# REEVALUATE/knowledge_enhanced_multimodal_retrieval

Measured on AMD Instinct MI355X. Metric: gallery images+texts encoded/sec (ViT-L/14; synthetic texts per SURVEY 8(d): end-of-text uniform in positions 8..76, mean 43.8 of 77 positions computed -- value_every_text_77_positions is the rate when every text fills the context) and 43k x Q sim+top-10 ms, higher is better.
Workload: dtype bf16; 1 GPU; CLIP ViT-L/14 zero-shot: 43k-gallery encode (1 image + query + target text per item, 224x224 / 77 tokens) + T2I top-10, BASELINE configs[1]; architecture=ViT-L/14, residual_stream=fp24, batch_per_gpu=255, text_group=1501, gallery=43000, parallelism=dp1 (gallery sharded), rccl_ranks=1

## Files before the change

include/kemr_debug.h:

```cpp
#ifndef KEMR_DEBUG_H_
#define KEMR_DEBUG_H_

#include <stddef.h>
#include <stdint.h>

#ifdef __cplusplus
extern "C" {
#endif

int kemr_debug_set(const char* key, int value);
int kemr_debug_get(const char* key, int* value);

int kemr_debug_sim_lists(const void* workspace_dev, int nq, int ng, int64_t kdim, int k, int32_t* out6);

int kemr_debug_gemm_stamps(unsigned* host_out, int n_words);

int kemr_debug_op_attention_packed(const void* qkv_dev, void* out_dev, const int* row_start_dev, int batch, int max_t, int width,
                                   void* stream);
int kemr_debug_op_attention_pooled(const void* q_dev, const void* qkv_dev, void* out_dev, const int* pool_idx_dev,
                                   const int* row_start_dev, int items, int tokens, int width, int causal, int force_long, void* stream);
int kemr_debug_op_tail(const void* x_dev, int x_dtype, const void* delta_dev, const void* delta2_dev, const int32_t* ids_dev,
                       const int* row_start_dev, int batch, int tokens, int width, const float* gamma_dev, const float* beta_dev,
                       const float* proj_dev, int d, int normalize, float* out_dev, void* stream);

int kemr_debug_image_tokens(struct kemr_model* m, const float* pixels_dev, int batch, float* out_dev, void* workspace_dev,
                            size_t workspace_bytes, void* stream);
int kemr_debug_text_tokens(struct kemr_model* m, const int32_t* ids_dev, const int32_t* lens_dev, int rows, int batch, void* out_dev,
                           int* row_start_out_dev, void* workspace_dev, size_t workspace_bytes, void* stream);

#ifdef __cplusplus
}
#endif
#endif
```

knowledge_enhanced_multimodal_retrieval_amd/_lib.py:

```python
from __future__ import annotations

import ctypes as C
import os
import threading

PKG_DIR = os.path.dirname(os.path.abspath(__file__))
LIB_PATH = os.path.join(PKG_DIR, "libkemr.so")

KEMR_F32, KEMR_BF16, KEMR_I32, KEMR_FP8 = 0, 1, 2, 3
KEMR_F24 = 24
PREC_BF16 = 1
PREC_BF16_RES16 = 2
PREC_FP8 = 3
PREC_FP8_MLP = 4
PREC_FP8_RES16 = 5
DEFAULT_PRECISION = "bf16-x24"
PRECISIONS = {"bf16": PREC_BF16, "bf16-res16": PREC_BF16_RES16, "fp8": PREC_FP8, "fp8-mlp": PREC_FP8_MLP, "fp8-res16": PREC_FP8_RES16,
              "bf16-x24": PREC_BF16, "fp8-x24": PREC_FP8}
TOWER_VISION, TOWER_TEXT = 0, 1
SIDE_QUERY, SIDE_GALLERY = 0, 1
EPI_BIAS_BF16, EPI_BIAS_QGELU_BF16, EPI_BIAS_RESID_F32 = 0, 1, 2
EPI_BIAS_RESADD_BF16 = 4
MAX_DEEP_K = 1024


class KemrCfg(C.Structure):
    _fields_ = [(n, C.c_int32) for n in ("embed_dim", "image_size", "patch", "v_width", "v_layers",
                                          "t_width", "t_layers", "vocab", "ctx")]


_vp, _i, _i64, _f, _sz = C.c_void_p, C.c_int, C.c_int64, C.c_float, C.c_size_t

SIGNATURES = {
    "kemr_last_error": (C.c_char_p, []),
    "kemr_abi_version": (_i, []),
    "kemr_model_create": (_i, [C.POINTER(KemrCfg), C.POINTER(_vp)]),
    "kemr_model_load_tensor": (_i, [_vp, C.c_char_p, _vp, _i, C.POINTER(_i64), _i]),
    "kemr_model_finalize": (_i, [_vp, _i]),
    "kemr_model_destroy": (_i, [_vp]),
    "kemr_model_set_option": (_i, [_vp, C.c_char_p, _i]),
    "kemr_model_get_option": (_i, [_vp, C.c_char_p, C.POINTER(_i)]),
    "kemr_model_num_tensors": (_i, [_vp]),
    "kemr_model_tensor_name": (C.c_char_p, [_vp, _i]),
    "kemr_workspace_bytes": (_sz, [_vp, _i, _i]),
    "kemr_encode_image": (_i, [_vp, _vp, _i, _vp, _i, _vp, _sz, _vp]),
    "kemr_encode_text": (_i, [_vp, _vp, _i, _vp, _i, _vp, _sz, _vp]),
    "kemr_text_packed_workspace_bytes": (_sz, [_vp, _i, _i]),
    "kemr_encode_text_packed": (_i, [_vp, _vp, _vp, _i, _i, _vp, _i, _vp, _sz, _vp]),
    "kemr_panel_kdim": (_i64, [_i, _i, _i]),
    "kemr_panel_build": (_i, [C.POINTER(_vp), C.POINTER(_f), C.POINTER(_vp), _i, _i, _i, _i, _i, _vp, _vp]),
    "kemr_sim_workspace_bytes": (_sz, [_i, _i, _i64, _i]),
    "kemr_sim_topk": (_i, [_vp, _i, _vp, _i, _i64, _i64, _i, _vp, _vp, _vp, _vp, _vp, _vp, _vp, _vp, _vp, _sz, _vp]),
    "kemr_pair_scores": (_i, [_vp, _vp, _i64, _vp, _vp, _i, _vp, _vp]),
    "kemr_topk_merge": (_i, [_vp, _vp, _i, _i, _i, _vp, _vp, _vp]),
    "kemr_scores_dense": (_i, [_vp, _i, _vp, _i, _i64, _vp, _i64, _vp]),
    "kemr_rank_dense": (_i, [_vp, _i, _i, _i64, _vp, _vp, _i, _vp, _vp, _vp]),
    "kemr_select_topk": (_i, [_vp, _vp, _i, _i, _i64, _i64, _i, _vp, _vp, _vp]),
    "kemr_sim_topk_deep_workspace_bytes": (_sz, [_i, _i, _i64, _i]),
    "kemr_sim_topk_deep": (_i, [_vp, _i, _vp, _i, _i64, _i64, _i, _vp, _vp, _vp, _sz, _vp]),
    "kemr_sim_topk_deep_fused": (_i, [_vp, _i, _vp, _i, _i64, _i64, _i, _vp, _vp, _vp, _vp, _vp, _vp, _vp, _vp, _vp, _sz, _vp]),
    "kemr_linear_head": (_i, [_vp, _vp, _i64, _vp, _vp, _vp, _f, _i, _vp, _vp]),
    "kemr_gate_rows": (_i, [_vp, _i, _i, _vp, _vp, _f, _i, _vp, _vp]),
    "kemr_cross_attention_pairs": (_i, [_vp, _vp, _vp, _vp, _vp, _vp, _vp, _vp, _f, _i, _i, _i, _i, _i, _vp, _vp]),
    "kemr_cross_attention_rerank": (_i, [_vp, _vp, _vp, _vp, _vp, _vp, _vp, _vp, _vp, _f, _i, _i, _i, _i, _i, _i, _vp, _i, _i64, _vp, _vp]),
    "kemr_profile_begin": (_i, [_i]),
    "kemr_profile_end": (_i, [C.POINTER(C.c_double), C.POINTER(_i64), _i]),
    "kemr_op_gemm": (_i, [_vp, _vp, _vp, _vp, _i, _i, _i, _i, _vp]),
    "kemr_preprocess_workspace_bytes": (_sz, [_i, _i, _i]),
    "kemr_preprocess_u8": (_i, [_vp, _i, _i, _i, _vp, _vp, _sz, _vp]),
    "kemr_preprocess_batch_workspace_bytes": (_sz, [_vp, _vp, _i, _i]),
    "kemr_preprocess_u8_batch": (_i, [_vp, _vp, _vp, _vp, _i, _i, _vp, _vp, _sz, _vp]),
    "kemr_op_gemm_fp8": (_i, [_vp, _vp, _vp, _vp, _vp, _i, _i, _i, _i, _vp]),
    "kemr_op_e4m3_host": (_i, [_vp, _vp, C.c_longlong]),
    "kemr_op_layernorm": (_i, [_vp, _vp, _vp, _vp, _i, _i, _i, _vp]),
    "kemr_op_layernorm_resid": (_i, [_vp, _vp, _vp, _vp, _vp, _i, _i, _vp]),
    "kemr_op_layernorm_rows": (_i, [_vp, _i, _vp, _vp, _i, _vp, _vp, _vp, _i, _i, _i, _vp]),
    "kemr_op_attention": (_i, [_vp, _vp, _i, _i, _i, _i, _vp]),
}

DEBUG_SIGNATURES = {
    "kemr_debug_set": (_i, [C.c_char_p, _i]),
    "kemr_debug_get": (_i, [C.c_char_p, C.POINTER(_i)]),
    "kemr_debug_sim_lists": (_i, [_vp, _i, _i, _i64, _i, _vp]),
    "kemr_debug_gemm_stamps": (_i, [_vp, _i]),
    "kemr_debug_op_attention_packed": (_i, [_vp, _vp, _vp, _i, _i, _i, _vp]),
    "kemr_debug_op_attention_pooled": (_i, [_vp, _vp, _vp, _vp, _vp, _i, _i, _i, _i, _i, _vp]),
    "kemr_debug_op_tail": (_i, [_vp, _i, _vp, _vp, _vp, _vp, _i, _i, _i, _vp, _vp, _vp, _i, _i, _vp, _vp]),
    "kemr_debug_image_tokens": (_i, [_vp, _vp, _i, _vp, _vp, _sz, _vp]),
    "kemr_debug_text_tokens": (_i, [_vp, _vp, _vp, _i, _i, _vp, _vp, _vp, _sz, _vp]),
}
ABI_VERSION = 4

_lock = threading.Lock()
_lib = None


def lib() -> C.CDLL:
    global _lib
    if _lib is not None:
        return _lib
    with _lock:
        if _lib is not None:
            return _lib
        if not os.path.exists(LIB_PATH):
            raise RuntimeError(
                f"{LIB_PATH} is missing: build it with `python -m knowledge_enhanced_multimodal_retrieval_amd.build` "
                "(hipcc, gfx950). There is no CPU fallback for this path.")
        import torch
        handle = C.CDLL(LIB_PATH)
        for name, (res, args) in list(SIGNATURES.items()) + list(DEBUG_SIGNATURES.items()):
            try:
                fn = getattr(handle, name)
            except AttributeError as e:
                raise RuntimeError(f"{LIB_PATH} does not export {name}; rebuild the library") from e
            fn.restype = res
            fn.argtypes = args
        if handle.kemr_abi_version() != ABI_VERSION:
            raise RuntimeError(f"libkemr.so ABI version {handle.kemr_abi_version()} != {ABI_VERSION}; rebuild the library")
        _lib = handle
        return _lib


def check(status: int, what: str = "") -> None:
    if status != 0:
        msg = lib().kemr_last_error()
        raise RuntimeError(f"libkemr {what} failed ({status}): {msg.decode() if msg else '?'}")
```

knowledge_enhanced_multimodal_retrieval_amd/csrc/api.hip:

```cpp
#include "common.h"
#include "../../include/kemr_debug.h"

#include <cmath>
#include <cstdarg>
#include <cstdio>
#include <cstring>
#include <map>
#include <string>
#include <vector>

namespace kemr {

static thread_local char g_err[512] = "";
void set_error(const char* fmt, ...) {
    va_list ap;
    va_start(ap, fmt);
    vsnprintf(g_err, sizeof(g_err), fmt, ap);
    va_end(ap);
}

struct ProfState {
    bool on = false;
    std::vector<hipEvent_t> ev;
    std::vector<int> cls;
    int used = 0;
};
static ProfState g_prof;

ProfScope::ProfScope(int c, hipStream_t s) : slot(-1), stream(s) {
    if (!g_prof.on || g_prof.used >= (int)g_prof.cls.size()) return;
    slot = g_prof.used++;
    g_prof.cls[slot] = c;
    (void)hipEventRecord(g_prof.ev[2 * slot], stream);
}
ProfScope::~ProfScope() {
    if (slot >= 0) (void)hipEventRecord(g_prof.ev[2 * slot + 1], stream);
}

struct HostTensor {
    std::vector<int64_t> shape;
    std::vector<float> data;
    bool loaded = false;
};

struct LayerW {
    const float *ln1_g, *ln1_b, *ln2_g, *ln2_b, *bqkv, *bo, *b1, *b2;
    const bf16_t *wqkv, *wo, *w1, *w2;
    const uint8_t *wqkv8 = nullptr, *w18 = nullptr;
    const float *sqkv = nullptr, *s1 = nullptr;
};

struct TowerW {
    int width = 0, layers = 0, tokens = 0;
    std::vector<LayerW> layer;
};

}

using namespace kemr;

struct kemr_model {
    kemr_cfg cfg;
    std::vector<std::string> names;
    std::map<std::string, HostTensor> tensors;
    bool finalized = false;
    char* arena = nullptr;
    size_t arena_bytes = 0;
    int grid = 0, patches = 0, kpad = 0;
    int res_dtype = KEMR_F32;
    int fp8 = 0;
    int resadd = 1;
    int last_pooled = 1;
    int stream24 = 1;
    TowerW vis;
    const bf16_t* conv_w = nullptr;
    const float *cls = nullptr, *vpos = nullptr, *lnpre_g = nullptr, *lnpre_b = nullptr, *lnpost_g = nullptr,
                *lnpost_b = nullptr, *vproj = nullptr;
    TowerW txt;
    const float *tok = nullptr, *tpos = nullptr, *lnf_g = nullptr, *lnf_b = nullptr, *tproj = nullptr;
};

namespace {

void add_block_names(std::vector<std::string>& v, std::map<std::string, HostTensor>& t, const std::string& prefix,
                     int width, int layers) {
    auto add = [&](const std::string& n, std::vector<int64_t> shape) { v.push_back(n); t[n].shape = std::move(shape); };
    for (int i = 0; i < layers; ++i) {
        const std::string b = prefix + ".resblocks." + std::to_string(i);
        add(b + ".ln_1.weight", {width});
        add(b + ".ln_1.bias", {width});
        add(b + ".attn.in_proj_weight", {3 * width, width});
        add(b + ".attn.in_proj_bias", {3 * width});
        add(b + ".attn.out_proj.weight", {width, width});
        add(b + ".attn.out_proj.bias", {width});
        add(b + ".ln_2.weight", {width});
        add(b + ".ln_2.bias", {width});
        add(b + ".mlp.c_fc.weight", {4 * width, width});
        add(b + ".mlp.c_fc.bias", {4 * width});
        add(b + ".mlp.c_proj.weight", {width, 4 * width});
        add(b + ".mlp.c_proj.bias", {width});
    }
}

int check_cfg(const kemr_cfg& c) {
    if (c.embed_dim <= 0 || c.embed_dim > 1024) KEMR_FAIL(KEMR_ERR_INVALID, "cfg: embed_dim %d not in 1..1024", c.embed_dim);
    if (c.patch <= 0 || c.image_size <= 0 || c.image_size % c.patch) KEMR_FAIL(KEMR_ERR_INVALID, "cfg: image_size %% patch != 0");
    if (c.v_width % 256 || c.t_width % 256 || c.v_width <= 0 || c.t_width <= 0 || c.v_width > 1280 || c.t_width > 1280)
        KEMR_FAIL(KEMR_ERR_INVALID, "cfg: widths must be multiples of 256 in 256..1280 (got %d, %d)", c.v_width, c.t_width);
    if (c.v_layers <= 0 || c.t_layers <= 0 || c.vocab <= 0 || c.ctx <= 0) KEMR_FAIL(KEMR_ERR_INVALID, "cfg: non-positive field");
    const int g = c.image_size / c.patch;
    if (c.ctx > KEMR_MAX_TEXT_CTX) KEMR_FAIL(KEMR_ERR_INVALID, "cfg: sequence length > 288 not supported");
    if ((int64_t)g * g + 1 > KEMR_MAX_VISION_TOKENS)
        KEMR_FAIL(KEMR_ERR_INVALID, "cfg: vision sequence length %lld > %d not supported", (long long)g * g + 1, KEMR_MAX_VISION_TOKENS);
    const int kpad = (int)round_up(3 * c.patch * c.patch, 64);
    if (kpad > 4 * c.v_width) KEMR_FAIL(KEMR_ERR_INVALID, "cfg: patch too large for the workspace layout");
    return KEMR_OK;
}

struct ArenaPlan {
    size_t bytes = 0;
    size_t take(size_t n) { size_t o = bytes; bytes += (size_t)round_up((int64_t)n, 256); return o; }
};

}

extern "C" const char* kemr_last_error(void) { return g_err; }
extern "C" int kemr_abi_version(void) { return KEMR_ABI_VERSION; }

extern "C" int kemr_model_create(const kemr_cfg* cfg, kemr_model** out) {
    if (!cfg || !out) KEMR_FAIL(KEMR_ERR_INVALID, "model_create: null argument");
    KEMR_TRY(check_cfg(*cfg));
    kemr_model* m = new (std::nothrow) kemr_model();
    if (!m) KEMR_FAIL(KEMR_ERR_NOMEM, "model_create: out of memory");
    m->cfg = *cfg;
    { const char* v = getenv("KEMR_RESADD"); const int e = (v && *v) ? atoi(v) : 1; m->resadd = e < 0 ? 0 : e > 2 ? 2 : e; }
    { const char* v = getenv("KEMR_LAST_BLOCK_FULL"); m->last_pooled = (v && *v && atoi(v) != 0) ? 0 : 1; }
    { const char* v = getenv("KEMR_STREAM24"); m->stream24 = (v && *v) ? (atoi(v) != 0 ? 1 : 0) : 1; }
    m->grid = cfg->image_size / cfg->patch;
    m->patches = m->grid * m->grid;
    m->kpad = (int)round_up(3 * cfg->patch * cfg->patch, 64);
    auto add = [&](const std::string& n, std::vector<int64_t> shape) { m->names.push_back(n); m->tensors[n].shape = std::move(shape); };
    const int vw = cfg->v_width, tw = cfg->t_width, D = cfg->embed_dim;
    add("visual.conv1.weight", {vw, 3, cfg->patch, cfg->patch});
    add("visual.class_embedding", {vw});
    add("visual.positional_embedding", {m->patches + 1, vw});
    add("visual.ln_pre.weight", {vw});
    add("visual.ln_pre.bias", {vw});
    add_block_names(m->names, m->tensors, "visual.transformer", vw, cfg->v_layers);
    add("visual.ln_post.weight", {vw});
    add("visual.ln_post.bias", {vw});
    add("visual.proj", {vw, D});
    add("token_embedding.weight", {cfg->vocab, tw});
    add("positional_embedding", {cfg->ctx, tw});
    add_block_names(m->names, m->tensors, "transformer", tw, cfg->t_layers);
    add("ln_final.weight", {tw});
    add("ln_final.bias", {tw});
    add("text_projection", {tw, D});
    *out = m;
    return KEMR_OK;
}

extern "C" int kemr_model_num_tensors(const kemr_model* m) { return m ? (int)m->names.size() : 0; }
extern "C" const char* kemr_model_tensor_name(const kemr_model* m, int i) {
    if (!m || i < 0 || i >= (int)m->names.size()) return nullptr;
    return m->names[i].c_str();
}

extern "C" int kemr_model_load_tensor(kemr_model* m, const char* name, const void* host_ptr, int dtype,
                                      const int64_t* shape, int rank) {
    if (!m || !name || !host_ptr || (!shape && rank > 0)) KEMR_FAIL(KEMR_ERR_INVALID, "load_tensor: null argument");
    if (dtype != KEMR_F32) KEMR_FAIL(KEMR_ERR_INVALID, "load_tensor(%s): only fp32 host tensors are accepted", name);
    const std::string n(name);
    if (n == "logit_scale" || n == "input_resolution" || n == "context_length" || n == "vocab_size") return KEMR_OK;
    auto it = m->tensors.find(n);
    if (it == m->tensors.end()) KEMR_FAIL(KEMR_ERR_INVALID, "load_tensor: unexpected key '%s' (strict load)", name);
    HostTensor& t = it->second;
    bool same = (int)t.shape.size() == rank;
    int64_t numel = 1;
    for (int i = 0; same && i < rank; ++i) same = t.shape[i] == shape[i];
    if (!same) {
        std::string want, got;
        for (auto s : t.shape) want += std::to_string(s) + ",";
        for (int i = 0; i < rank; ++i) got += std::to_string(shape[i]) + ",";
        KEMR_FAIL(KEMR_ERR_INVALID, "load_tensor: size mismatch for %s: expected [%s] got [%s]", name, want.c_str(), got.c_str());
    }
    for (auto s : t.shape) numel *= s;
    t.data.assign((const float*)host_ptr, (const float*)host_ptr + numel);
    t.loaded = true;
    m->finalized = false;
    return KEMR_OK;
}

extern "C" int kemr_model_finalize(kemr_model* m, int precision) {
    if (!m) KEMR_FAIL(KEMR_ERR_INVALID, "finalize: null model");
    if (precision < KEMR_PREC_BF16 || precision > KEMR_PREC_FP8_RES16)
        KEMR_FAIL(KEMR_ERR_INVALID, "finalize: unsupported precision %d", precision);
    const int fp8 = (precision == KEMR_PREC_FP8 || precision == KEMR_PREC_FP8_RES16) ? 1 : precision == KEMR_PREC_FP8_MLP ? 3 : 0;
    if (fp8 && ((m->cfg.v_width % 128) || (m->cfg.t_width % 128) || m->cfg.v_width < 256 || m->cfg.t_width < 256))
        KEMR_FAIL(KEMR_ERR_INVALID, "finalize: fp8 needs tower widths that are multiples of 128 and >= 256");
    for (const auto& n : m->names)
        if (!m->tensors[n].loaded) KEMR_FAIL(KEMR_ERR_STATE, "finalize: missing key '%s' (strict load)", n.c_str());

    ArenaPlan plan;
    std::map<std::string, size_t> off;
    auto is_matrix = [](const std::string& n) {
        return n.find("in_proj_weight") != std::string::npos || n.find("out_proj.weight") != std::string::npos ||
               n.find("c_fc.weight") != std::string::npos || n.find("c_proj.weight") != std::string::npos ||
               n == "visual.conv1.weight";
    };
    auto is_fp8_matrix = [&](const std::string& n) {
        if (n.rfind("visual.", 0) != 0) return false;
        return ((fp8 & 1) && n.find("in_proj_weight") != std::string::npos) || ((fp8 & 2) && n.find("c_fc.weight") != std::string::npos);
    };
    for (const auto& n : m->names) {
        const HostTensor& t = m->tensors[n];
        size_t bytes;
        if (n == "visual.conv1.weight") bytes = (size_t)m->cfg.v_width * m->kpad * 2;
        else if (is_fp8_matrix(n)) { bytes = t.data.size(); off[n + "#scale"] = plan.take((size_t)t.shape[0] * 4); }
        else if (is_matrix(n)) bytes = t.data.size() * 2;
        else bytes = t.data.size() * 4;
        off[n] = plan.take(bytes);
    }
    auto ends_with = [](const std::string& a, const char* suf) { const size_t k = strlen(suf); return a.size() >= k && !a.compare(a.size() - k, k, suf); };
    auto ln_of = [&](const std::string& n) -> std::string {
        const size_t p = n.find(".attn.in_proj_weight");
        if (p != std::string::npos) return n.substr(0, p) + ".ln_1";
        const size_t q = n.find(".mlp.c_fc.weight");
        return q != std::string::npos ? n.substr(0, q) + ".ln_2" : std::string();
    };
    std::map<std::string, std::vector<float>> a_scale;
    if (fp8)
        for (const auto& n : m->names)
            if (is_fp8_matrix(n)) {
                const std::string ln = ln_of(n);
                const std::vector<float>&g = m->tensors[ln + ".weight"].data, &bb = m->tensors[ln + ".bias"].data;
                std::vector<float> sc(g.size(), 1.0f);
                for (size_t c = 0; c < g.size(); ++c) {
                    const float a = fmaxf(fabsf(g[c]), fabsf(bb[c]));
                    if (a > 0.f && std::isfinite(a)) sc[c] = exp2f(fminf(12.f, fmaxf(-12.f, ceilf(log2f(a)))));
                }
                a_scale[ln] = sc;
            }
    std::vector<char> host(plan.bytes, 0);
    for (const auto& n : m->names) {
        const HostTensor& t = m->tensors[n];
        char* dst = host.data() + off[n];
        if (n == "visual.conv1.weight") {
            const int kv = 3 * m->cfg.patch * m->cfg.patch;
            bf16_t* d = (bf16_t*)dst;
            for (int r = 0; r < m->cfg.v_width; ++r)
                for (int k = 0; k < kv; ++k) d[(size_t)r * m->kpad + k] = f32_to_bf16_host(t.data[(size_t)r * kv + k]);
        } else if (is_fp8_matrix(n)) {
            const int64_t rows = t.shape[0], cols = t.shape[1];
            const bool qkv = n.find("in_proj_weight") != std::string::npos;
            const std::vector<float>& as = a_scale.at(ln_of(n));
            uint8_t* d = (uint8_t*)dst;
            float* sc = (float*)(host.data() + off[n + "#scale"]);
            for (int64_t r = 0; r < rows; ++r) {
                const float pre = (qkv && r < cols) ? 0.125f : 1.0f;
                float amax = 0.f;
                for (int64_t c = 0; c < cols; ++c) amax = fmaxf(amax, fabsf(t.data[r * cols + c] * pre * as[c]));
                const float scale = amax > 0.f ? amax / 448.f : 1.0f;
                sc[r] = scale;
                for (int64_t c = 0; c < cols; ++c) d[r * cols + c] = f32_to_e4m3_host(t.data[r * cols + c] * pre * as[c] / scale);
            }
        } else if (n.find("in_proj_weight") != std::string::npos) {
            const int64_t w = t.shape[1];
            bf16_t* d = (bf16_t*)dst;
            for (int64_t i = 0; i < (int64_t)t.data.size(); ++i)
                d[i] = f32_to_bf16_host(i < w * w ? t.data[i] * 0.125f : t.data[i]);
        } else if (n.find("in_proj_bias") != std::string::npos) {
            const int64_t w = t.shape[0] / 3;
            float* d = (float*)dst;
            for (int64_t i = 0; i < (int64_t)t.data.size(); ++i) d[i] = i < w ? t.data[i] * 0.125f : t.data[i];
        } else if (is_matrix(n)) {
            bf16_t* d = (bf16_t*)dst;
            for (size_t i = 0; i < t.data.size(); ++i) d[i] = f32_to_bf16_host(t.data[i]);
        } else if (fp8 && (ends_with(n, ".ln_1.weight") || ends_with(n, ".ln_1.bias") || ends_with(n, ".ln_2.weight") || ends_with(n, ".ln_2.bias")) &&
                   a_scale.count(n.substr(0, n.rfind('.')))) {
            const std::vector<float>& as = a_scale.at(n.substr(0, n.rfind('.')));
            float* d = (float*)dst;
            for (size_t c = 0; c < t.data.size(); ++c) d[c] = t.data[c] / as[c];
        } else {
            memcpy(dst, t.data.data(), t.data.size() * 4);
        }
    }
    if (m->arena && m->arena_bytes != plan.bytes) { (void)hipFree(m->arena); m->arena = nullptr; }
    if (!m->arena) {
        KEMR_CHECK_HIP(hipMalloc((void**)&m->arena, plan.bytes));
        m->arena_bytes = plan.bytes;
    }
    KEMR_CHECK_HIP(hipDeviceSynchronize());
    KEMR_CHECK_HIP(hipMemcpy(m->arena, host.data(), plan.bytes, hipMemcpyHostToDevice));

    auto F = [&](const std::string& n) { return (const float*)(m->arena + off.at(n)); };
    auto H = [&](const std::string& n) { return (const bf16_t*)(m->arena + off.at(n)); };
    auto tower = [&](TowerW& tw, const std::string& prefix, int width, int layers, int tokens, int fp8) {
        tw.width = width; tw.layers = layers; tw.tokens = tokens;
        tw.layer.resize(layers);
        for (int i = 0; i < layers; ++i) {
            const std::string b = prefix + ".resblocks." + std::to_string(i);
            LayerW& L = tw.layer[i];
            L.ln1_g = F(b + ".ln_1.weight"); L.ln1_b = F(b + ".ln_1.bias");
            L.wqkv = H(b + ".attn.in_proj_weight"); L.bqkv = F(b + ".attn.in_proj_bias");
            if (fp8 & 1) { L.wqkv8 = (const uint8_t*)L.wqkv; L.wqkv = nullptr; L.sqkv = F(b + ".attn.in_proj_weight#scale"); }
            if (fp8 & 2) { L.w18 = (const uint8_t*)H(b + ".mlp.c_fc.weight"); L.s1 = F(b + ".mlp.c_fc.weight#scale"); }
            L.wo = H(b + ".attn.out_proj.weight"); L.bo = F(b + ".attn.out_proj.bias");
            L.ln2_g = F(b + ".ln_2.weight"); L.ln2_b = F(b + ".ln_2.bias");
            L.w1 = (fp8 & 2) ? nullptr : H(b + ".mlp.c_fc.weight"); L.b1 = F(b + ".mlp.c_fc.bias");
            L.w2 = H(b + ".mlp.c_proj.weight"); L.b2 = F(b + ".mlp.c_proj.bias");
        }
    };
    tower(m->vis, "visual.transformer", m->cfg.v_width, m->cfg.v_layers, m->patches + 1, fp8);
    tower(m->txt, "transformer", m->cfg.t_width, m->cfg.t_layers, m->cfg.ctx, 0);
    m->conv_w = H("visual.conv1.weight");
    m->cls = F("visual.class_embedding"); m->vpos = F("visual.positional_embedding");
    m->lnpre_g = F("visual.ln_pre.weight"); m->lnpre_b = F("visual.ln_pre.bias");
    m->lnpost_g = F("visual.ln_post.weight"); m->lnpost_b = F("visual.ln_post.bias");
    m->vproj = F("visual.proj");
    m->tok = F("token_embedding.weight"); m->tpos = F("positional_embedding");
    m->lnf_g = F("ln_final.weight"); m->lnf_b = F("ln_final.bias"); m->tproj = F("text_projection");

    for (auto& kv : m->tensors) { std::vector<float>().swap(kv.second.data); kv.second.loaded = false; }
    m->res_dtype = (precision == KEMR_PREC_BF16_RES16 || precision == KEMR_PREC_FP8_RES16) ? KEMR_BF16 : KEMR_F32;
    if (m->stream24 && m->res_dtype == KEMR_F32) m->res_dtype = KEMR_F24;
    m->fp8 = fp8;
    m->finalized = true;
    return KEMR_OK;
}

extern "C" int kemr_model_destroy(kemr_model* m) {
    if (!m) return KEMR_OK;
    if (m->arena) (void)hipFree(m->arena);
    delete m;
    return KEMR_OK;
}

namespace {

struct Workspace {
    void* x;
    int x_dtype;
    bf16_t* h;
    bf16_t* big;
    bf16_t* delta;
    bf16_t* delta2;
    float* x32;
    int* pool_idx;
    void* xc;
    bf16_t *hc, *qc, *ac, *d1c, *d2c;
    bf16_t* gc;
};

size_t compact_bytes(int width, int items) {
    const int64_t Mc = round_up((int64_t)items, 256);
    return (size_t)(round_up((int64_t)items * 4, 256) + Mc * width * 4 + 5 * Mc * width * 2 + Mc * width * 8);
}

size_t ws_bytes_rows(int width, int64_t rows, int x_dtype) {
    const int64_t Mp = round_up(rows, 256);
    const int xb = x_dtype == KEMR_BF16 ? 2 : (x_dtype == KEMR_F24 ? 3 : 4);
    return (size_t)(round_up(Mp * width * xb, 256) + 3 * round_up(Mp * width * 2, 256) + round_up(Mp * width * 8, 256));
}

size_t ws_bytes(int width, int tokens, int batch, int x_dtype) {
    const int64_t Mp = round_up((int64_t)batch * tokens, 256);
    const int xb = x_dtype == KEMR_BF16 ? 2 : (x_dtype == KEMR_F24 ? 3 : 4);
    return (size_t)(round_up(Mp * width * xb, 256) + 3 * round_up(Mp * width * 2, 256) + round_up(Mp * width * 8, 256));
}

int carve(Workspace& w, void* base, size_t bytes, int width, int64_t rows, int items, int x_dtype) {
    const size_t need = ws_bytes_rows(width, rows, x_dtype) + compact_bytes(width, items);
    if (!base || bytes < need) KEMR_FAIL(KEMR_ERR_WORKSPACE, "workspace too small: %zu < %zu bytes", bytes, need);
    if ((uintptr_t)base % 256) KEMR_FAIL(KEMR_ERR_WORKSPACE, "workspace must be 256-byte aligned");
    const int64_t Mp = round_up(rows, 256);
    char* p = (char*)base;
    w.x = p; w.x_dtype = x_dtype; p += round_up(Mp * width * (x_dtype == KEMR_BF16 ? 2 : (x_dtype == KEMR_F24 ? 3 : 4)), 256);
    w.x32 = x_dtype == KEMR_F32 ? (float*)w.x : (float*)p;
    w.h = (bf16_t*)p; p += round_up(Mp * width * 2, 256);
    w.delta = (bf16_t*)p; p += round_up(Mp * width * 2, 256);
    w.delta2 = (bf16_t*)p; p += round_up(Mp * width * 2, 256);
    w.big = (bf16_t*)p; p += round_up(Mp * width * 8, 256);
    const int64_t Mc = round_up((int64_t)items, 256);
    w.pool_idx = (int*)p; p += round_up((int64_t)items * 4, 256);
    w.xc = p; p += Mc * width * 4;
    w.hc = (bf16_t*)p; p += Mc * width * 2;
    w.qc = (bf16_t*)p; p += Mc * width * 2;
    w.ac = (bf16_t*)p; p += Mc * width * 2;
    w.d1c = (bf16_t*)p; p += Mc * width * 2;
    w.d2c = (bf16_t*)p; p += Mc * width * 2;
    w.gc = (bf16_t*)p;
    return KEMR_OK;
}

int run_blocks(const TowerW& t, const Workspace& w, int batch, int causal, int fp8, int want_resadd, hipStream_t s, bool* pending,
               const int* row_start = nullptr, int rows = 0, int last_pooled = 0, const int32_t* ids = nullptr, bool* compact = nullptr) {
    const int W = t.width, M = row_start ? rows : batch * t.tokens;
    const bool fq = fp8 & 1, f1 = fp8 & 2;
    bool resadd = want_resadd >= (w.x_dtype == KEMR_BF16 ? 1 : 2) && M > 512 && W % 256 == 0 && w.x_dtype != KEMR_F24;
    const int cs = w.x_dtype == KEMR_BF16 ? 2 : 4;
    const int epi_res = w.x_dtype == KEMR_BF16 ? EPI_BIAS_RESADD_BF16 : EPI_BIAS_RESID_F32;
    if (resadd) {
        GemmParams a{}, b{};
        a.M = b.M = M; a.N = b.N = W; a.K = W; b.K = 4 * W; a.lda = W; b.lda = 4 * W; a.ldw = W; b.ldw = 4 * W; a.ldc = b.ldc = W;
        a.c_rows_padded = b.c_rows_padded = 1;
        resadd = gemm256u_fits(a, 2, cs) && gemm256u_fits(b, 2, cs);
    }
    *pending = !resadd && t.layers > 0;
    const bool pooled = last_pooled && compact && !resadd && !f1 && t.layers > 0 && t.tokens <= KEMR_MAX_VISION_TOKENS;
    if (compact) *compact = pooled;
    if (pooled) KEMR_TRY(launch_pool_index(causal ? ids : nullptr, row_start, batch, t.tokens, w.pool_idx, s));
    for (int l = 0; l < t.layers; ++l) {
        const LayerW& L = t.layer[l];
        if (pooled && l == t.layers - 1) {
            KEMR_TRY(launch_layernorm(w.x, w.x_dtype, l ? w.delta : nullptr, l ? w.delta2 : nullptr, 1, L.ln1_g, L.ln1_b, w.h, M, W, fq ? KEMR_FP8 : KEMR_BF16, s));
            GemmParams g{};
            g.c_rows_padded = 1;
            g.M = M; g.A = w.h; g.lda = W; g.ldw = W; g.bias = L.bqkv + W; g.C = w.big + W; g.ldc = 3 * W; g.N = 2 * W; g.K = W;
            if (fq) { g.W = (const bf16_t*)(L.wqkv8 + (size_t)W * W); g.wscale = L.sqkv + W; KEMR_TRY(launch_gemm256u_fp8(g, EPI_BIAS_BF16, s)); }
            else { g.W = L.wqkv + (size_t)W * W; KEMR_TRY(launch_gemm(g, EPI_BIAS_BF16, s)); }
            KEMR_TRY(launch_gather_pooled(w.x, w.x_dtype, w.h, fq ? KEMR_FP8 : KEMR_BF16, w.pool_idx, batch, W, w.xc, w.hc, s));
            g.M = batch; g.A = w.hc; g.bias = L.bqkv; g.C = w.qc; g.ldc = W; g.N = W;
            if (fq) { g.W = (const bf16_t*)L.wqkv8; g.wscale = L.sqkv; KEMR_TRY(launch_gemm256u_fp8(g, EPI_BIAS_BF16, s)); g.wscale = nullptr; }
            else { g.W = L.wqkv; KEMR_TRY(launch_gemm(g, EPI_BIAS_BF16, s)); }
            KEMR_TRY(launch_attention_pooled(w.qc, w.big, w.ac, w.pool_idx, row_start, batch, t.tokens, W, causal, s));
            g.A = w.ac; g.W = L.wo; g.bias = L.bo; g.C = w.d1c;
            KEMR_TRY(launch_gemm(g, EPI_BIAS_BF16, s));
            KEMR_TRY(launch_layernorm(w.xc, w.x_dtype, w.d1c, nullptr, 0, L.ln2_g, L.ln2_b, w.hc, batch, W, KEMR_BF16, s));
            g.A = w.hc; g.W = L.w1; g.bias = L.b1; g.C = w.gc; g.ldc = 4 * W; g.N = 4 * W;
            KEMR_TRY(launch_gemm(g, EPI_BIAS_QGELU_BF16, s));
            g.A = w.gc; g.lda = 4 * W; g.W = L.w2; g.ldw = 4 * W; g.bias = L.b2; g.C = w.d2c; g.ldc = W; g.N = W; g.K = 4 * W;
            KEMR_TRY(launch_gemm(g, EPI_BIAS_BF16, s));
            break;
        }
        if (resadd) KEMR_TRY(launch_layernorm(w.x, w.x_dtype, nullptr, nullptr, 0, L.ln1_g, L.ln1_b, w.h, M, W, fq ? KEMR_FP8 : KEMR_BF16, s));
        else KEMR_TRY(launch_layernorm(w.x, w.x_dtype, l ? w.delta : nullptr, l ? w.delta2 : nullptr, 1, L.ln1_g, L.ln1_b, w.h, M, W, fq ? KEMR_FP8 : KEMR_BF16, s));
        GemmParams g{};
        g.M = M;
        g.c_rows_padded = 1;
        g.A = w.h; g.lda = W; g.W = L.wqkv; g.ldw = W; g.bias = L.bqkv; g.C = w.big; g.ldc = 3 * W; g.N = 3 * W; g.K = W;
        if (fq) {
            g.W = (const bf16_t*)L.wqkv8; g.wscale = L.sqkv;
            KEMR_TRY(launch_gemm256u_fp8(g, EPI_BIAS_BF16, s));
            g.wscale = nullptr;
        } else {
            KEMR_TRY(launch_gemm(g, EPI_BIAS_BF16, s));
        }
        if (row_start) KEMR_TRY(launch_attention_packed(w.big, w.h, row_start, batch, t.tokens, W, s));
        else KEMR_TRY(launch_attention(w.big, w.h, batch, t.tokens, W, causal, s));
        g.A = w.h; g.lda = W; g.W = L.wo; g.ldw = W; g.bias = L.bo; g.C = resadd ? w.x : (void*)w.delta; g.ldc = W; g.N = W; g.K = W;
        KEMR_TRY(launch_gemm(g, resadd ? epi_res : EPI_BIAS_BF16, s));
        KEMR_TRY(launch_layernorm(w.x, w.x_dtype, resadd ? nullptr : w.delta, nullptr, 0, L.ln2_g, L.ln2_b, w.h, M, W, f1 ? KEMR_FP8 : KEMR_BF16, s));
        g.A = w.h; g.lda = W; g.W = L.w1; g.ldw = W; g.bias = L.b1; g.C = w.big; g.ldc = 4 * W; g.N = 4 * W; g.K = W;
        if (f1) {
            g.W = (const bf16_t*)L.w18; g.wscale = L.s1;
            KEMR_TRY(launch_gemm256u_fp8(g, EPI_BIAS_QGELU_BF16, s));
            g.wscale = nullptr;
        } else {
            KEMR_TRY(launch_gemm(g, EPI_BIAS_QGELU_BF16, s));
        }
        g.A = w.big; g.lda = 4 * W; g.W = L.w2; g.ldw = 4 * W; g.bias = L.b2; g.C = resadd ? w.x : (void*)w.delta2; g.ldc = W; g.N = W; g.K = 4 * W;
        KEMR_TRY(launch_gemm(g, resadd ? epi_res : EPI_BIAS_BF16, s));
    }
    return KEMR_OK;
}

int image_front(kemr_model* m, const float* pixels_dev, int batch, const void* out_dev, void* workspace_dev, size_t workspace_bytes,
                hipStream_t s, const char* what, Workspace& w) {
    if (!m || !pixels_dev || !out_dev) KEMR_FAIL(KEMR_ERR_INVALID, "%s: null argument", what);
    if (!m->finalized) KEMR_FAIL(KEMR_ERR_STATE, "%s: model not finalized", what);
    if (batch <= 0) return batch == 0 ? KEMR_OK : (set_error("%s: negative batch", what), KEMR_ERR_INVALID);
    if ((int64_t)batch * (m->patches + 1) > (1 << 24)) KEMR_FAIL(KEMR_ERR_INVALID, "%s: batch %d too large", what, batch);
    const int W = m->cfg.v_width, T = m->patches + 1;
    KEMR_TRY(carve(w, workspace_dev, workspace_bytes, W, (int64_t)batch * T, batch, m->res_dtype));
    KEMR_TRY(launch_im2col(pixels_dev, w.big, batch, m->cfg.image_size, m->cfg.patch, m->kpad, s));
    GemmParams g{};
    g.A = w.big; g.lda = m->kpad; g.W = m->conv_w; g.ldw = m->kpad; g.bias = nullptr; g.C = w.x32; g.ldc = W;
    g.pos = m->vpos; g.patches = m->patches; g.M = batch * m->patches; g.N = W; g.K = m->kpad;
    KEMR_TRY(launch_gemm(g, EPI_PATCH_F32, s));
    return launch_cls_rows(w.x32, m->cls, m->vpos, batch, T, W, s);
}

int text_front(kemr_model* m, const int32_t* ids_dev, const int32_t* lens_dev, int rows, int batch, bool packed, const void* out_dev,
               void* workspace_dev, size_t workspace_bytes, hipStream_t s, const char* what, Workspace& w, int** row_start) {
    if (!m || !ids_dev || !out_dev || (packed && !lens_dev)) KEMR_FAIL(KEMR_ERR_INVALID, "%s: null argument", what);
    if (!m->finalized) KEMR_FAIL(KEMR_ERR_STATE, "%s: model not finalized", what);
    if (batch <= 0) return batch == 0 ? KEMR_OK : (set_error("%s: negative batch", what), KEMR_ERR_INVALID);
    if ((int64_t)batch * m->cfg.ctx > (1 << 24)) KEMR_FAIL(KEMR_ERR_INVALID, "%s: batch %d too large", what, batch);
    const int W = m->cfg.t_width, T = m->cfg.ctx;
    *row_start = nullptr;
    if (!packed) {
        KEMR_TRY(carve(w, workspace_dev, workspace_bytes, W, (int64_t)batch * T, batch, m->res_dtype));
        return launch_text_embed(ids_dev, m->tok, m->tpos, w.x, w.x_dtype, batch, T, W, m->cfg.vocab, s);
    }
    if (m->cfg.ctx > 128) KEMR_FAIL(KEMR_ERR_INVALID, "%s: context length %d > 128", what, m->cfg.ctx);
    if (rows < batch || (int64_t)rows > (int64_t)batch * T) KEMR_FAIL(KEMR_ERR_INVALID, "%s: %d rows for %d texts of 1 .. %d positions", what, rows, batch, T);
    const size_t base_bytes = ws_bytes_rows(W, rows, m->res_dtype) + compact_bytes(W, batch), need = base_bytes + (size_t)round_up(((int64_t)batch + 1) * 4, 256);
    if (workspace_bytes < need) KEMR_FAIL(KEMR_ERR_WORKSPACE, "workspace too small: %zu < %zu bytes", workspace_bytes, need);
    KEMR_TRY(carve(w, workspace_dev, workspace_bytes, W, rows, batch, m->res_dtype));
    *row_start = (int*)((char*)workspace_dev + base_bytes);
    KEMR_TRY(launch_row_starts(lens_dev, batch, T, rows, *row_start, s));
    return launch_text_embed(ids_dev, m->tok, m->tpos, w.x, w.x_dtype, batch, T, W, m->cfg.vocab, s, *row_start, rows);
}

}

extern "C" size_t kemr_workspace_bytes(const kemr_model* m, int tower, int batch) {
    if (!m || batch <= 0) return 0;
    if (tower == KEMR_TOWER_VISION) return ws_bytes(m->cfg.v_width, m->patches + 1, batch, m->res_dtype) + compact_bytes(m->cfg.v_width, batch);
    if (tower == KEMR_TOWER_TEXT) return ws_bytes(m->cfg.t_width, m->cfg.ctx, batch, m->res_dtype) + compact_bytes(m->cfg.t_width, batch);
    return 0;
}

extern "C" size_t kemr_text_packed_workspace_bytes(const kemr_model* m, int rows, int batch) {
    if (!m || batch <= 0 || rows < batch) return 0;
    return ws_bytes_rows(m->cfg.t_width, rows, m->res_dtype) + compact_bytes(m->cfg.t_width, batch) +
           (size_t)round_up(((int64_t)batch + 1) * 4, 256);
}

extern "C" int kemr_encode_image(kemr_model* m, const float* pixels_dev, int batch, float* out_dev, int normalize,
                                 void* workspace_dev, size_t workspace_bytes, void* stream) {
    hipStream_t s = (hipStream_t)stream;
    Workspace w;
    KEMR_TRY(image_front(m, pixels_dev, batch, out_dev, workspace_dev, workspace_bytes, s, "encode_image", w));
    if (batch == 0) return KEMR_OK;
    const int W = m->cfg.v_width, T = m->patches + 1;
    KEMR_TRY(launch_layernorm(w.x32, KEMR_F32, nullptr, nullptr, 0, m->lnpre_g, m->lnpre_b, w.x, batch * T, W, w.x_dtype, s));
    bool vb = false, vc = false;
    KEMR_TRY(run_blocks(m->vis, w, batch, 0, m->fp8, m->resadd, s, &vb, nullptr, 0, m->last_pooled, nullptr, &vc));
    if (vc) KEMR_TRY(launch_tail(w.xc, w.x_dtype, w.d1c, w.d2c, nullptr, batch, 1, W, m->lnpost_g, m->lnpost_b, m->vproj, m->cfg.embed_dim, normalize, out_dev, s));
    else KEMR_TRY(launch_tail(w.x, w.x_dtype, vb ? w.delta : nullptr, vb ? w.delta2 : nullptr, nullptr, batch, T, W, m->lnpost_g, m->lnpost_b, m->vproj, m->cfg.embed_dim, normalize, out_dev, s));
    return KEMR_OK;
}

extern "C" int kemr_encode_text(kemr_model* m, const int32_t* ids_dev, int batch, float* out_dev, int normalize,
                                void* workspace_dev, size_t workspace_bytes, void* stream) {
    hipStream_t s = (hipStream_t)stream;
    Workspace w;
    int* no_rows = nullptr;
    KEMR_TRY(text_front(m, ids_dev, nullptr, 0, batch, false, out_dev, workspace_dev, workspace_bytes, s, "encode_text", w, &no_rows));
    if (batch == 0) return KEMR_OK;
    const int W = m->cfg.t_width, T = m->cfg.ctx;
    bool tb = false, tc = false;
    KEMR_TRY(run_blocks(m->txt, w, batch, 1, 0, m->resadd, s, &tb, nullptr, 0, m->last_pooled, ids_dev, &tc));
    if (tc) KEMR_TRY(launch_tail(w.xc, w.x_dtype, w.d1c, w.d2c, nullptr, batch, 1, W, m->lnf_g, m->lnf_b, m->tproj, m->cfg.embed_dim, normalize, out_dev, s));
    else KEMR_TRY(launch_tail(w.x, w.x_dtype, tb ? w.delta : nullptr, tb ? w.delta2 : nullptr, ids_dev, batch, T, W, m->lnf_g, m->lnf_b, m->tproj, m->cfg.embed_dim, normalize, out_dev, s));
    return KEMR_OK;
}

extern "C" int kemr_encode_text_packed(kemr_model* m, const int32_t* ids_dev, const int32_t* lens_dev, int rows, int batch, float* out_dev,
                                       int normalize, void* workspace_dev, size_t workspace_bytes, void* stream) {
    hipStream_t s = (hipStream_t)stream;
    Workspace w;
    int* row_start = nullptr;
    KEMR_TRY(text_front(m, ids_dev, lens_dev, rows, batch, true, out_dev, workspace_dev, workspace_bytes, s, "encode_text_packed", w, &row_start));
    if (batch == 0) return KEMR_OK;
    const int W = m->cfg.t_width, T = m->cfg.ctx;
    bool tb = false, tc = false;
    KEMR_TRY(run_blocks(m->txt, w, batch, 1, 0, m->resadd, s, &tb, row_start, rows, m->last_pooled, ids_dev, &tc));
    if (tc) KEMR_TRY(launch_tail(w.xc, w.x_dtype, w.d1c, w.d2c, nullptr, batch, 1, W, m->lnf_g, m->lnf_b, m->tproj, m->cfg.embed_dim, normalize, out_dev, s));
    else KEMR_TRY(launch_tail(w.x, w.x_dtype, tb ? w.delta : nullptr, tb ? w.delta2 : nullptr, ids_dev, batch, T, W, m->lnf_g, m->lnf_b, m->tproj, m->cfg.embed_dim, normalize, out_dev, s, row_start));
    return KEMR_OK;
}

extern "C" int kemr_model_set_option(kemr_model* m, const char* key, int value) {
    if (!m || !key) KEMR_FAIL(KEMR_ERR_INVALID, "model_set_option: null argument");
    if (!strcmp(key, "residual_fusion")) {
        if (value < 0 || value > 2) KEMR_FAIL(KEMR_ERR_INVALID, "model_set_option(residual_fusion): 0, 1 or 2, got %d", value);
        m->resadd = value;
        return KEMR_OK;
    }
    if (!strcmp(key, "residual_stream_24bit")) {
        if (value < 0 || value > 1) KEMR_FAIL(KEMR_ERR_INVALID, "model_set_option(residual_stream_24bit): 0 or 1, got %d", value);
        if (m->finalized) KEMR_FAIL(KEMR_ERR_STATE, "model_set_option(residual_stream_24bit): set it before kemr_model_finalize");
        m->stream24 = value;
        return KEMR_OK;
    }
    if (!strcmp(key, "last_block_pooled_row")) {
        if (value < 0 || value > 1) KEMR_FAIL(KEMR_ERR_INVALID, "model_set_option(last_block_pooled_row): 0 or 1, got %d", value);
        m->last_pooled = value;
        return KEMR_OK;
    }
    KEMR_FAIL(KEMR_ERR_INVALID, "model_set_option: unknown key '%s'", key);
}

extern "C" int kemr_model_get_option(const kemr_model* m, const char* key, int* value) {
    if (!m || !key || !value) KEMR_FAIL(KEMR_ERR_INVALID, "model_get_option: null argument");
    if (!strcmp(key, "residual_fusion")) { *value = m->resadd; return KEMR_OK; }
    if (!strcmp(key, "last_block_pooled_row")) { *value = m->last_pooled; return KEMR_OK; }
    if (!strcmp(key, "residual_stream_24bit")) { *value = m->finalized ? (m->res_dtype == KEMR_F24) : m->stream24; return KEMR_OK; }
    if (!strcmp(key, "precision_residual_bf16")) { *value = m->res_dtype == KEMR_BF16; return KEMR_OK; }
    KEMR_FAIL(KEMR_ERR_INVALID, "model_get_option: unknown key '%s'", key);
}

namespace {
#ifdef KEMR_AB_VARIANTS
int g_ab_variants = 1;
#else
int g_ab_variants = 0;
#endif
struct DebugKnob { const char* key; int* var; int lo, hi; unsigned product; };
int* sim_lists_knob();
const DebugKnob* debug_knobs(int* n) {
    static const DebugKnob knobs[] = {
        {"gemm_variant", &g_gemm_variant, 0, 9, 1u << 0 | 1u << 1 | 1u << 2 | 1u << 7 | 1u << 8},
        {"gemm_flags", &g_gemm_dbg, 0, 255, 1u << 0},
        {"gemm_order", &g_gemm_order, 0, 8, ~0u},
        {"gemm_grid", &g_gemm_grid, 0, 1024, ~0u},
        {"gemm_conc", &g_gemm_conc, 0, 2, ~0u},
        {"gemm_kl", &g_gemm_kl, 0, 1, 1u << 0},
        {"attn_v", &g_attn_v, 0, 5, 1u << 0},
        {"attn_xcd", &g_attn_xcd, 0, 1, ~0u},
        {"attn_waves", &g_attn_waves, 0, 8, 1u << 0},
        {"ln_nt", &g_ln_nt, 0, 3, 1u << 3},
        {"sim_lists", sim_lists_knob(), 0, 3, ~0u},
        {"ab_variants", &g_ab_variants, -1, -2, 0},
    };
    *n = (int)(sizeof(knobs) / sizeof(knobs[0]));
    return knobs;
}
int* sim_lists_knob() { return &g_sim_lists; }
}

extern "C" int kemr_debug_set(const char* key, int value) {
    if (!key) KEMR_FAIL(KEMR_ERR_INVALID, "debug_set: null key");
    int n = 0;
    const DebugKnob* k = debug_knobs(&n);
    for (int i = 0; i < n; ++i)
        if (!strcmp(k[i].key, key)) {
            if (k[i].lo > k[i].hi) KEMR_FAIL(KEMR_ERR_INVALID, "debug_set(%s): read-only", key);
            if (value < k[i].lo || value > k[i].hi) KEMR_FAIL(KEMR_ERR_INVALID, "debug_set(%s): %d not in %d..%d", key, value, k[i].lo, k[i].hi);
            if (!g_ab_variants && !(value < 32 && ((k[i].product >> value) & 1u)) && k[i].product != ~0u)
                KEMR_FAIL(KEMR_ERR_INVALID, "debug_set(%s): %d selects an A/B experiment kernel that is not in this library (build.py --ab-variants)", key, value);
            *k[i].var = value;
            return KEMR_OK;
        }
    KEMR_FAIL(KEMR_ERR_INVALID, "debug_set: unknown key '%s'", key);
}

extern "C" int kemr_debug_get(const char* key, int* value) {
    if (!key || !value) KEMR_FAIL(KEMR_ERR_INVALID, "debug_get: null argument");
    int n = 0;
    const DebugKnob* k = debug_knobs(&n);
    for (int i = 0; i < n; ++i)
        if (!strcmp(k[i].key, key)) { *value = *k[i].var; return KEMR_OK; }
    KEMR_FAIL(KEMR_ERR_INVALID, "debug_get: unknown key '%s'", key);
}

extern "C" int kemr_debug_gemm_stamps(unsigned* host_out, int n_words) {
    if (!host_out) KEMR_FAIL(KEMR_ERR_INVALID, "debug_gemm_stamps: null output");
    return gemm_read_stamps(host_out, n_words);
}

extern "C" int kemr_debug_op_attention_packed(const void* qkv_dev, void* out_dev, const int* row_start_dev, int batch, int max_t, int width,
                                              void* stream) {
    if (!qkv_dev || !out_dev) KEMR_FAIL(KEMR_ERR_INVALID, "debug_op_attention_packed: null argument");
    return launch_attention_packed((const bf16_t*)qkv_dev, (bf16_t*)out_dev, row_start_dev, batch, max_t, width, (hipStream_t)stream);
}

extern "C" int kemr_debug_op_attention_pooled(const void* q_dev, const void* qkv_dev, void* out_dev, const int* pool_idx_dev,
                                              const int* row_start_dev, int items, int tokens, int width, int causal, int force_long,
                                              void* stream) {
    if (!q_dev || !qkv_dev || !out_dev) KEMR_FAIL(KEMR_ERR_INVALID, "debug_op_attention_pooled: null argument");
    return launch_attention_pooled((const bf16_t*)q_dev, (const bf16_t*)qkv_dev, (bf16_t*)out_dev, pool_idx_dev, row_start_dev, items,
                                   tokens, width, causal, (hipStream_t)stream, force_long);
}

extern "C" int kemr_debug_op_tail(const void* x_dev, int x_dtype, const void* delta_dev, const void* delta2_dev, const int32_t* ids_dev,
                                  const int* row_start_dev, int batch, int tokens, int width, const float* gamma_dev, const float* beta_dev,
                                  const float* proj_dev, int d, int normalize, float* out_dev, void* stream) {
    if (!x_dev || !gamma_dev || !beta_dev || !proj_dev || !out_dev) KEMR_FAIL(KEMR_ERR_INVALID, "debug_op_tail: null argument");
    if (x_dtype != KEMR_F32 && x_dtype != KEMR_BF16 && x_dtype != KEMR_F24) KEMR_FAIL(KEMR_ERR_INVALID, "debug_op_tail: bad row dtype %d", x_dtype);
    return launch_tail(x_dev, x_dtype, (const bf16_t*)delta_dev, (const bf16_t*)delta2_dev, ids_dev, batch, tokens, width, gamma_dev, beta_dev,
                       proj_dev, d, normalize, out_dev, (hipStream_t)stream, row_start_dev);
}

extern "C" int kemr_debug_image_tokens(kemr_model* m, const float* pixels_dev, int batch, float* out_dev, void* workspace_dev,
                                       size_t workspace_bytes, void* stream) {
    hipStream_t s = (hipStream_t)stream;
    Workspace w;
    KEMR_TRY(image_front(m, pixels_dev, batch, out_dev, workspace_dev, workspace_bytes, s, "debug_image_tokens", w));
    if (batch == 0) return KEMR_OK;
    const size_t bytes = (size_t)batch * (m->patches + 1) * m->cfg.v_width * 4;
    KEMR_CHECK_HIP(hipMemcpyAsync(out_dev, w.x32, bytes, hipMemcpyDeviceToDevice, s));
    return KEMR_OK;
}

extern "C" int kemr_debug_text_tokens(kemr_model* m, const int32_t* ids_dev, const int32_t* lens_dev, int rows, int batch, void* out_dev,
                                      int* row_start_out_dev, void* workspace_dev, size_t workspace_bytes, void* stream) {
    const bool packed = lens_dev != nullptr;
    if (packed && !row_start_out_dev) KEMR_FAIL(KEMR_ERR_INVALID, "debug_text_tokens: null row_start output");
    hipStream_t s = (hipStream_t)stream;
    Workspace w;
    int* row_start = nullptr;
    KEMR_TRY(text_front(m, ids_dev, lens_dev, rows, batch, packed, out_dev, workspace_dev, workspace_bytes, s, "debug_text_tokens", w, &row_start));
    if (batch == 0) return KEMR_OK;
    const int xb = w.x_dtype == KEMR_BF16 ? 2 : (w.x_dtype == KEMR_F24 ? 3 : 4);
    const int64_t n = packed ? rows : (int64_t)batch * m->cfg.ctx;
    KEMR_CHECK_HIP(hipMemcpyAsync(out_dev, w.x, (size_t)n * m->cfg.t_width * xb, hipMemcpyDeviceToDevice, s));
    if (packed) KEMR_CHECK_HIP(hipMemcpyAsync(row_start_out_dev, row_start, ((size_t)batch + 1) * 4, hipMemcpyDeviceToDevice, s));
    return KEMR_OK;
}

extern "C" int kemr_profile_begin(int max_launches) {
    if (max_launches <= 0 || max_launches > (1 << 20)) KEMR_FAIL(KEMR_ERR_INVALID, "profile_begin: bad max_launches");
    if (g_prof.on) KEMR_FAIL(KEMR_ERR_STATE, "profile_begin: already profiling");
    while ((int)g_prof.ev.size() < 2 * max_launches) {
        hipEvent_t e;
        KEMR_CHECK_HIP(hipEventCreate(&e));
        g_prof.ev.push_back(e);
    }
    g_prof.cls.assign(max_launches, 0);
    g_prof.used = 0;
    g_prof.on = true;
    return KEMR_OK;
}

extern "C" int kemr_profile_end(double* ms_per_class, int64_t* launches_per_class, int nclass) {
    if (!g_prof.on) KEMR_FAIL(KEMR_ERR_STATE, "profile_end: not profiling");
    g_prof.on = false;
    if (!ms_per_class || !launches_per_class || nclass < PROF_NCLASS) KEMR_FAIL(KEMR_ERR_INVALID, "profile_end: need %d classes", PROF_NCLASS);
    for (int i = 0; i < nclass; ++i) { ms_per_class[i] = 0; launches_per_class[i] = 0; }
    KEMR_CHECK_HIP(hipDeviceSynchronize());
    for (int i = 0; i < g_prof.used; ++i) {
        float ms = 0.f;
        KEMR_CHECK_HIP(hipEventElapsedTime(&ms, g_prof.ev[2 * i], g_prof.ev[2 * i + 1]));
        ms_per_class[g_prof.cls[i]] += ms;
        launches_per_class[g_prof.cls[i]] += 1;
    }
    return KEMR_OK;
}

extern "C" int kemr_op_gemm(const void* a_dev, const void* w_dev, const float* bias_dev, void* c_dev, int m, int n, int k,
                            int epilogue, void* stream) {
    if (!a_dev || !w_dev || !c_dev) KEMR_FAIL(KEMR_ERR_INVALID, "op_gemm: null argument");
    if (epilogue < 0 || (epilogue > KEMR_EPI_BIAS_RESID_F32 && epilogue != KEMR_EPI_BIAS_RESADD_BF16)) KEMR_FAIL(KEMR_ERR_INVALID, "op_gemm: bad epilogue %d", epilogue);
    GemmParams g{};
    g.A = (const bf16_t*)a_dev; g.lda = k; g.W = (const bf16_t*)w_dev; g.ldw = k; g.bias = bias_dev; g.C = c_dev; g.ldc = n;
    g.M = m; g.N = n; g.K = k;
    g.c_rows_padded = 1;
    return launch_gemm(g, epilogue, (hipStream_t)stream);
}

extern "C" int kemr_op_gemm_fp8(const void* a_dev, const void* w_dev, const float* wscale_dev, const float* bias_dev, void* c_dev,
                                int m, int n, int k, int epilogue, void* stream) {
    if (!a_dev || !w_dev || !wscale_dev || !c_dev) KEMR_FAIL(KEMR_ERR_INVALID, "op_gemm_fp8: null argument");
    GemmParams g{};
    g.A = (const bf16_t*)a_dev; g.lda = k; g.W = (const bf16_t*)w_dev; g.ldw = k; g.bias = bias_dev; g.wscale = wscale_dev;
    g.C = c_dev; g.ldc = n; g.M = m; g.N = n; g.K = k;
    g.c_rows_padded = 1;
    return launch_gemm256u_fp8(g, epilogue, (hipStream_t)stream);
}

extern "C" int kemr_op_e4m3_host(const float* in, unsigned char* out, long long n) {
    if (!in || !out || n < 0) KEMR_FAIL(KEMR_ERR_INVALID, "op_e4m3_host: bad argument");
    for (long long i = 0; i < n; ++i) out[i] = f32_to_e4m3_host(in[i]);
    return KEMR_OK;
}

extern "C" int kemr_op_layernorm(const float* x_dev, const float* gamma_dev, const float* beta_dev, void* y_dev, int rows,
                                 int width, int out_dtype, void* stream) {
    if (!x_dev || !gamma_dev || !beta_dev || !y_dev) KEMR_FAIL(KEMR_ERR_INVALID, "op_layernorm: null argument");
    return launch_layernorm((void*)x_dev, KEMR_F32, nullptr, nullptr, 0, gamma_dev, beta_dev, y_dev, rows, width, out_dtype, (hipStream_t)stream);
}

extern "C" int kemr_op_layernorm_resid(float* x_dev, const void* delta_dev, const float* gamma_dev, const float* beta_dev,
                                       void* y_dev, int rows, int width, void* stream) {
    if (!x_dev || !delta_dev || !gamma_dev || !beta_dev || !y_dev) KEMR_FAIL(KEMR_ERR_INVALID, "op_layernorm_resid: null argument");
    return launch_layernorm(x_dev, KEMR_F32, (const bf16_t*)delta_dev, nullptr, 1, gamma_dev, beta_dev, y_dev, rows, width, KEMR_BF16, (hipStream_t)stream);
}

extern "C" int kemr_op_layernorm_rows(void* x_dev, int x_dtype, const void* delta_dev, const void* delta2_dev, int writeback,
                                      const float* gamma_dev, const float* beta_dev, void* y_dev, int rows, int width,
                                      int out_dtype, void* stream) {
    if (!x_dev || !gamma_dev || !beta_dev || !y_dev) KEMR_FAIL(KEMR_ERR_INVALID, "op_layernorm_rows: null argument");
    return launch_layernorm(x_dev, x_dtype, (const bf16_t*)delta_dev, (const bf16_t*)delta2_dev, writeback, gamma_dev, beta_dev,
                            y_dev, rows, width, out_dtype, (hipStream_t)stream);
}

extern "C" int kemr_op_attention(const void* qkv_dev, void* out_dev, int batch, int t, int width, int causal, void* stream) {
    if (!qkv_dev || !out_dev) KEMR_FAIL(KEMR_ERR_INVALID, "op_attention: null argument");
    return launch_attention((const bf16_t*)qkv_dev, (bf16_t*)out_dev, batch, t, width, causal, (hipStream_t)stream);
}
```

knowledge_enhanced_multimodal_retrieval_amd/csrc/attention.hip:

```cpp
#include "common.h"

namespace kemr {

__device__ __forceinline__ bf16x4 lds_read_tr16(const char* p) {
    typedef __attribute__((ext_vector_type(4))) short s4;
    return __builtin_amdgcn_ds_read_tr16_b64_v4i16((__attribute__((address_space(3))) s4*)p);
}

__device__ __forceinline__ bool attn_item(int xbatch, int& h, int& b) {
    h = blockIdx.x; b = blockIdx.y;
    if (xbatch == 0) return true;
    const int id = blockIdx.y * gridDim.x + blockIdx.x, j = id >> 3;
    b = (j / (int)gridDim.x) * 8 + (id & 7);
    h = j % (int)gridDim.x;
    return b < xbatch;
}

#ifndef KEMR_ATTN_PRIO
#define KEMR_ATTN_PRIO 0
#endif
__device__ __forceinline__ void attn_prio(int mfma_phase) {
    if constexpr (KEMR_ATTN_PRIO == 1) { if (mfma_phase) __builtin_amdgcn_s_setprio(1); else __builtin_amdgcn_s_setprio(0); }
    if constexpr (KEMR_ATTN_PRIO == 2) { if (mfma_phase) __builtin_amdgcn_s_setprio(0); else __builtin_amdgcn_s_setprio(1); }
}

template <bool NT>
__device__ __forceinline__ bf16x8 load_q8(const bf16_t* p) {
    if constexpr (NT) return __builtin_nontemporal_load((const bf16x8*)p);
    else return *(const bf16x8*)p;
}

template <int NT32, bool CAUSAL, int TC, int NW = 4, bool STAMP = false, int NTLOAD = 1, bool SKIPTAIL = false>
__global__ __launch_bounds__(NW * 64, 2) void attention_kernel(const bf16_t* __restrict__ qkv, bf16_t* __restrict__ out,
                                                           int T_rt, int width, int xbatch, const int* __restrict__ row_start) {
    constexpr int TP = NT32 * 32;
    constexpr int NT16 = NT32 * 2;
    constexpr int NTH = NW * 64;
    constexpr int NCH = (TP * 8 + NTH - 1) / NTH;
    constexpr float LOG2E = 1.4426950408889634f;
    extern __shared__ __attribute__((aligned(16))) char smem[];
    char* sK = smem;
    char* sV = smem + TP * 128;

    int h, b;
    if (!attn_item(xbatch, h, b)) return;
    int T_ = TC > 0 ? TC : T_rt;
    size_t row0 = (size_t)b * T_;
    if (TC == 0 && row_start) {
        const int r0 = row_start[b];
        T_ = row_start[b + 1] - r0;
        row0 = r0;
    }
    const int T = T_;
    const int tid = threadIdx.x, lane = tid & 63;
    const int wid = __builtin_amdgcn_readfirstlane(tid >> 6);
    const int ld = 3 * width;
    const bf16_t* base = qkv + row0 * ld + h * 64;
    const int lrow = lane & 15, lq = lane >> 4;
    const int nqt = SKIPTAIL ? T >> 4 : (T + 15) >> 4;

    unsigned long long st_t[8] = {0, 0, 0, 0, 0, 0, 0, 0}, st_prev = 0;
    auto stamp = [&](int k) {
        if constexpr (STAMP) {
            __builtin_amdgcn_sched_barrier(0);
            unsigned long long now;
            asm volatile("s_memtime %0\n\ts_waitcnt lgkmcnt(0)" : "=s"(now) :: "memory");
            __builtin_amdgcn_sched_barrier(0);
            st_t[k] += now - st_prev;
            st_prev = now;
        }
    };
    if constexpr (STAMP) { asm volatile("s_memtime %0\n\ts_waitcnt lgkmcnt(0)" : "=s"(st_prev) :: "memory"); __builtin_amdgcn_sched_barrier(0); }
    bf16x8 qn[2];
    {
        const int q0 = wid * 16 + lrow;
        const int qc = q0 < T ? q0 : T - 1;
#pragma unroll
        for (int kk = 0; kk < 2; ++kk) qn[kk] = load_q8<(NTLOAD >= 2)>(base + (size_t)qc * ld + kk * 32 + lq * 8);
    }
    {
        uint4 kv[NCH], vv[NCH];
#pragma unroll
        for (int i = 0; i < NCH; ++i) {
            const int idx = tid + i * NTH;
            const int row = idx >> 3, c = idx & 7;
            const int rc = row < T ? row : T - 1;
            if constexpr (NTLOAD >= 1) {
                typedef unsigned u32x4_ __attribute__((ext_vector_type(4)));
                const u32x4_ a_ = __builtin_nontemporal_load((const u32x4_*)(base + (size_t)rc * ld + width + c * 8));
                const u32x4_ b_ = __builtin_nontemporal_load((const u32x4_*)(base + (size_t)rc * ld + 2 * width + c * 8));
                kv[i] = make_uint4(a_.x, a_.y, a_.z, a_.w);
                vv[i] = make_uint4(b_.x, b_.y, b_.z, b_.w);
            } else {
                kv[i] = *(const uint4*)(base + (size_t)rc * ld + width + c * 8);
                vv[i] = *(const uint4*)(base + (size_t)rc * ld + 2 * width + c * 8);
            }
        }
#pragma unroll
        for (int i = 0; i < NCH; ++i) {
            const int idx = tid + i * NTH;
            const int row = idx >> 3, c = idx & 7;
            if (idx < TP * 8) {
                const unsigned keep = row < T ? 0xffffffffu : 0u;
                uint4 a = kv[i], b2 = vv[i];
                a.x &= keep; a.y &= keep; a.z &= keep; a.w &= keep;
                b2.x &= keep; b2.y &= keep; b2.z &= keep; b2.w &= keep;
                *(uint4*)(sK + row * 128 + ((c ^ ((row >> 1) & 7)) << 4)) = a;
                *(uint4*)(sV + row * 128 + ((c ^ (((row >> 1) & 3) << 1)) << 4)) = b2;
            }
        }
    }
    __syncthreads();
    stamp(0);

    for (int qt = wid; qt < nqt; qt += NW) {
        const int q = qt * 16 + lrow;
        bf16x8 qf[2] = {qn[0], qn[1]};
        if (qt + NW < nqt) {
            const int q2 = q + NW * 16;
            const int qc = q2 < T ? q2 : T - 1;
#pragma unroll
            for (int kk = 0; kk < 2; ++kk) qn[kk] = load_q8<(NTLOAD >= 2)>(base + (size_t)qc * ld + kk * 32 + lq * 8);
        }

        constexpr int G = (NT16 % 3 == 0) ? 3 : 2;
        constexpr int NG = NT16 / G;
        f32x4 s[NT16];
        bf16x8 kfr[2][G][2];
        auto load_group = [&](int g, bf16x8 (&dst)[G][2]) {
#pragma unroll
            for (int j = 0; j < G; ++j)
#pragma unroll
                for (int kk = 0; kk < 2; ++kk)
                    dst[j][kk] = *(const bf16x8*)(sK + ((g * G + j) * 16 + lrow) * 128 + (((kk * 4 + lq) ^ (lrow >> 1)) << 4));
        };
        load_group(0, kfr[0]);
        attn_prio(1);
#pragma unroll
        for (int g = 0; g < NG; ++g) {
            if (g + 1 < NG && (g + 1) * G * 16 < T) load_group(g + 1, kfr[(g + 1) & 1]);
            __builtin_amdgcn_sched_barrier(0);
#pragma unroll
            for (int j = 0; j < G; ++j) {
                const int t = g * G + j;
                s[t] = f32x4{0.f, 0.f, 0.f, 0.f};
                if (t * 16 < T && (!CAUSAL || t <= qt)) {
                    s[t] = __builtin_amdgcn_mfma_f32_16x16x32_bf16(kfr[g & 1][j][0], qf[0], s[t], 0, 0, 0);
                    s[t] = __builtin_amdgcn_mfma_f32_16x16x32_bf16(kfr[g & 1][j][1], qf[1], s[t], 0, 0, 0);
                }
            }
            __builtin_amdgcn_sched_barrier(0);
        }
        attn_prio(0);
        stamp(1);
        float mx = -INFINITY;
#pragma unroll
        for (int t = 0; t < NT16; ++t) {
            const bool partial = (t + 1) * 16 > T || CAUSAL;
#pragma unroll
            for (int r = 0; r < 4; ++r) {
                if (partial) {
                    const int key = t * 16 + lq * 4 + r;
                    const bool ok = key < T && (!CAUSAL || key <= q);
                    s[t][r] = ok ? s[t][r] : -INFINITY;
                }
                mx = fmaxf(mx, s[t][r]);
            }
        }
        mx = fmaxf(mx, __shfl_xor(mx, 16));
        mx = fmaxf(mx, __shfl_xor(mx, 32));
        const float mxl = mx * LOG2E;
        stamp(2);
        f32x2_t sum2 = {0.f, 0.f};
        const f32x2_t l2 = {LOG2E, LOG2E}, nm = {-mxl, -mxl};
        auto exp_tile = [&](int t) {
            f32x2_t a = f32x2_t{s[t][0], s[t][1]} * l2 + nm, c = f32x2_t{s[t][2], s[t][3]} * l2 + nm;
            a.x = __builtin_amdgcn_exp2f(a.x); a.y = __builtin_amdgcn_exp2f(a.y);
            c.x = __builtin_amdgcn_exp2f(c.x); c.y = __builtin_amdgcn_exp2f(c.y);
            s[t][0] = a.x; s[t][1] = a.y; s[t][2] = c.x; s[t][3] = c.y;
            sum2 += a;
            sum2 += c;
        };
#pragma unroll
        for (int t = 0; t < NT16; ++t) exp_tile(t);

        stamp(3);
        f32x4 o[4];
#pragma unroll
        for (int dt = 0; dt < 4; ++dt) o[dt] = f32x4{0.f, 0.f, 0.f, 0.f};
        bf16x8 vfr[2][4];
        auto load_v = [&](int u, bf16x8 (&dst)[4]) {
            const int ra = u * 32 + lq * 4 + (lrow >> 2);
            const int rb = ra + 16;
#pragma unroll
            for (int dt = 0; dt < 4; ++dt) {
                const int c = dt * 2 + ((lrow & 3) >> 1);
                const bf16x4 va = lds_read_tr16(sV + ra * 128 + ((c ^ (((ra >> 1) & 3) << 1)) << 4) + (lrow & 1) * 8);
                const bf16x4 vb = lds_read_tr16(sV + rb * 128 + ((c ^ (((rb >> 1) & 3) << 1)) << 4) + (lrow & 1) * 8);
                dst[dt][0] = va[0]; dst[dt][1] = va[1]; dst[dt][2] = va[2]; dst[dt][3] = va[3];
                dst[dt][4] = vb[0]; dst[dt][5] = vb[1]; dst[dt][6] = vb[2]; dst[dt][7] = vb[3];
            }
        };
        load_v(0, vfr[0]);
        attn_prio(1);
        auto live = [&](int u) { return u < NT32 && u * 32 < T && !(CAUSAL && u * 32 > qt * 16 + 15); };
#pragma unroll
        for (int u = 0; u < NT32; ++u) {
            if (!live(u)) continue;
            if (u + 1 < NT32 && (u + 1) * 32 < T) load_v(u + 1, vfr[(u + 1) & 1]);
            __builtin_amdgcn_sched_barrier(0);
            union { bf16x8 v; uint32_t w[4]; } pf;
            pf.w[0] = pack_bf16x2(s[2 * u][0], s[2 * u][1]);
            pf.w[1] = pack_bf16x2(s[2 * u][2], s[2 * u][3]);
            pf.w[2] = pack_bf16x2(s[2 * u + 1][0], s[2 * u + 1][1]);
            pf.w[3] = pack_bf16x2(s[2 * u + 1][2], s[2 * u + 1][3]);
#pragma unroll
            for (int dt = 0; dt < 4; ++dt)
                o[dt] = __builtin_amdgcn_mfma_f32_16x16x32_bf16(vfr[u & 1][dt], pf.v, o[dt], 0, 0, 0);
            __builtin_amdgcn_sched_barrier(0);
        }
        attn_prio(0);
        stamp(4);
        float sum = sum2.x + sum2.y;
        sum += __shfl_xor(sum, 16);
        sum += __shfl_xor(sum, 32);
        if (q < T) {
            const float inv = 1.0f / sum;
            bf16_t* dst = out + (row0 + q) * width + h * 64 + lq * 4;
#pragma unroll
            for (int dt = 0; dt < 4; ++dt) {
                uint2 pk;
                pk.x = pack_bf16x2(o[dt][0] * inv, o[dt][1] * inv);
                pk.y = pack_bf16x2(o[dt][2] * inv, o[dt][3] * inv);
                *(uint2*)(dst + dt * 16) = pk;
            }
        }
        stamp(5);
    }
    if constexpr (STAMP) {
        unsigned long long* dst = (unsigned long long*)(out + (size_t)xbatch * T * width) + (((size_t)b * (width >> 6) + h) * NW + wid) * 8;
        if (lane == 0) {
#pragma unroll
            for (int k = 0; k < 6; ++k) dst[k] += st_t[k];
            dst[6] += 1;
        }
    }
}

int g_attn_v = 0;

int g_attn_xcd = 1;
int g_attn_waves = 0;

#ifdef KEMR_AB_VARIANTS
int launch_attention_ab(int v, int waves, const bf16_t* qkv, bf16_t* out, int batch, int width, int xbatch, hipStream_t stream);
#endif

template <int NT32>
static int launch_nt(const bf16_t* qkv, bf16_t* out, int batch, int t, int width, int causal, hipStream_t stream, const int* row_start = nullptr) {
    constexpr int smem = NT32 * 32 * 128 * 2;
    const dim3 grid(width / 64, batch);
    ProfScope prof(PROF_ATTENTION, stream);
    void (*kern)(const bf16_t*, bf16_t*, int, int, int, const int*);
    const int xbatch = g_attn_xcd ? batch : 0;
    const dim3 xgrid(width / 64, xbatch ? (batch + 7) / 8 * 8 : batch);
    int threads = 256;
    if (causal) {
        if (NT32 == 3 && t == 77 && !row_start) { kern = attention_kernel<NT32, true, NT32 == 3 ? 77 : 0, NT32 == 3 ? 5 : 4>; threads = 320; }
        else kern = attention_kernel<NT32, true, 0>;
    } else if (NT32 == 9 && t == 257) {
#ifdef KEMR_AB_VARIANTS
        if (g_attn_v != 0) return launch_attention_ab(g_attn_v, g_attn_waves, qkv, out, batch, width, xbatch, stream);
        if (g_attn_waves == 6) { kern = attention_kernel<NT32, false, NT32 == 9 ? 257 : 0, NT32 == 9 ? 6 : 4>; threads = 384; }
        else if (g_attn_waves == 7) kern = attention_kernel<NT32, false, NT32 == 9 ? 257 : 0, 4, false, NT32 == 9 ? 0 : 1>;
        else if (g_attn_waves == 8) kern = attention_kernel<NT32, false, NT32 == 9 ? 257 : 0, 4, false, 1, NT32 == 9>;
        else if (g_attn_waves == 5) kern = attention_kernel<NT32, false, NT32 == 9 ? 257 : 0, 4, false, NT32 == 9 ? 2 : 1>;
        else if (g_attn_waves == 2 && xbatch) kern = attention_kernel<NT32, false, NT32 == 9 ? 257 : 0, 4, NT32 == 9>;
        else
#else
        if (g_attn_v != 0 || g_attn_waves != 0)
            KEMR_FAIL(KEMR_ERR_INVALID, "attention: attn_v = %d / attn_waves = %d select A/B kernels this library was built without (build.py --ab-variants)", g_attn_v, g_attn_waves);
#endif
        kern = attention_kernel<NT32, false, NT32 == 9 ? 257 : 0>;
    } else {
        kern = attention_kernel<NT32, false, 0>;
    }
    KEMR_CHECK_HIP(hipFuncSetAttribute((const void*)kern, hipFuncAttributeMaxDynamicSharedMemorySize, smem));
    hipLaunchKernelGGL(kern, xgrid, dim3(threads), smem, stream, qkv, out, t, width, xbatch, row_start);
    KEMR_CHECK_LAUNCH("attention_kernel");
    return KEMR_OK;
}

int launch_attention(const bf16_t* qkv, bf16_t* out, int batch, int t, int width, int causal, hipStream_t stream) {
    if (batch <= 0) return KEMR_OK;
    if (width % 64 != 0 || t <= 0) KEMR_FAIL(KEMR_ERR_INVALID, "attention: bad shape t=%d width=%d", t, width);
    if (batch > 65528) KEMR_FAIL(KEMR_ERR_INVALID, "attention: batch %d > 65528 (grid.y, rounded up to a multiple of 8)", batch);
    const int nt32 = (t + 31) / 32;
    switch (nt32) {
        case 1: return launch_nt<1>(qkv, out, batch, t, width, causal, stream);
        case 2: return launch_nt<2>(qkv, out, batch, t, width, causal, stream);
        case 3: return launch_nt<3>(qkv, out, batch, t, width, causal, stream);
        case 4: return launch_nt<4>(qkv, out, batch, t, width, causal, stream);
        case 5: return launch_nt<5>(qkv, out, batch, t, width, causal, stream);
        case 6: return launch_nt<6>(qkv, out, batch, t, width, causal, stream);
        case 7: return launch_nt<7>(qkv, out, batch, t, width, causal, stream);
        case 8: return launch_nt<8>(qkv, out, batch, t, width, causal, stream);
        case 9: return launch_nt<9>(qkv, out, batch, t, width, causal, stream);
    }
    if (!causal && t <= KEMR_MAX_VISION_TOKENS) return launch_attention_long(qkv, out, batch, t, width, stream);
    if (!causal) KEMR_FAIL(KEMR_ERR_INVALID, "attention: sequence length %d > %d not supported", t, KEMR_MAX_VISION_TOKENS);
    KEMR_FAIL(KEMR_ERR_INVALID, "attention: sequence length %d > 288 not supported (causal)", t);
}

__device__ __forceinline__ void wave_lds_fence() {
    __builtin_amdgcn_fence(__ATOMIC_RELEASE, "wavefront");
    __builtin_amdgcn_wave_barrier();
    __builtin_amdgcn_fence(__ATOMIC_ACQUIRE, "wavefront");
}

template <int MAXK>
__global__ __launch_bounds__(256) void attention_pooled_kernel(const bf16_t* __restrict__ q, const bf16_t* __restrict__ qkv,
                                                               bf16_t* __restrict__ out, const int* __restrict__ pool_idx,
                                                               const int* __restrict__ row_start, int items, int tokens, int width,
                                                               int causal) {
    constexpr float LOG2E = 1.4426950408889634f;
    __shared__ float sp[4][MAXK];
    const int heads = width >> 6, lane = threadIdx.x & 63, wv = threadIdx.x >> 6;
    const int item = blockIdx.x * 4 + wv;
    if (item >= items * heads) return;
    const int b = item / heads, h = item - b * heads;
    const int r0 = row_start ? row_start[b] : b * tokens;
    int nk = causal ? pool_idx[b] - r0 + 1 : tokens;
    nk = nk < 1 ? 1 : (nk > MAXK ? MAXK : nk);
    const size_t ld = 3 * (size_t)width;
    const int ck = lane & 7, kq = lane >> 3;
    float qf[8];
    {
        const uint4 v = ((const uint4*)(q + (size_t)b * width + h * 64))[ck];
        const uint32_t w4[4] = {v.x, v.y, v.z, v.w};
#pragma unroll
        for (int k = 0; k < 4; ++k) {
            qf[2 * k] = bf16_to_f32((bf16_t)(w4[k] & 0xffff));
            qf[2 * k + 1] = bf16_to_f32((bf16_t)(w4[k] >> 16));
        }
    }
    const bf16_t* kbase = qkv + (size_t)r0 * ld + width + h * 64 + ck * 8;
    const int npass = (nk + 7) >> 3;
    for (int pss = 0; pss < npass; ++pss) {
        const int j = pss * 8 + kq;
        const int jc = j < nk ? j : nk - 1;
        const uint4 v = *(const uint4*)(kbase + (size_t)jc * ld);
        const uint32_t w4[4] = {v.x, v.y, v.z, v.w};
        float s = 0.f;
#pragma unroll
        for (int k = 0; k < 4; ++k) {
            s = fmaf(qf[2 * k], bf16_to_f32((bf16_t)(w4[k] & 0xffff)), s);
            s = fmaf(qf[2 * k + 1], bf16_to_f32((bf16_t)(w4[k] >> 16)), s);
        }
        s += __shfl_xor(s, 1);
        s += __shfl_xor(s, 2);
        s += __shfl_xor(s, 4);
        if (ck == 0 && j < nk) sp[wv][j] = s;
    }
    wave_lds_fence();
    float sc[MAXK / 64];
    float mx = -INFINITY;
#pragma unroll
    for (int pss = 0; pss < MAXK / 64; ++pss) {
        const int j = pss * 64 + lane;
        sc[pss] = j < nk ? sp[wv][j] : -INFINITY;
        mx = fmaxf(mx, sc[pss]);
    }
#pragma unroll
    for (int o = 32; o > 0; o >>= 1) mx = fmaxf(mx, __shfl_xor(mx, o));
    float sum = 0.f;
#pragma unroll
    for (int pss = 0; pss < MAXK / 64; ++pss) {
        const int j = pss * 64 + lane;
        const float p = __builtin_amdgcn_exp2f((sc[pss] - mx) * LOG2E);
        sum += p;
        if (j < MAXK) sp[wv][j] = bf16_to_f32(f32_to_bf16(p));
    }
#pragma unroll
    for (int o = 32; o > 0; o >>= 1) sum += __shfl_xor(sum, o);
    wave_lds_fence();
    const int dp = lane & 31, par = lane >> 5;
    const bf16_t* vp = qkv + (size_t)r0 * ld + 2 * width + h * 64 + dp * 2;
    float a0 = 0.f, a1 = 0.f;
#pragma unroll 4
    for (int j = par; j < nk; j += 2) {
        const uint32_t v = *(const uint32_t*)(vp + (size_t)j * ld);
        const float p = sp[wv][j];
        a0 = fmaf(p, bf16_to_f32((bf16_t)(v & 0xffff)), a0);
        a1 = fmaf(p, bf16_to_f32((bf16_t)(v >> 16)), a1);
    }
    a0 += __shfl_xor(a0, 32);
    a1 += __shfl_xor(a1, 32);
    if (par == 0) {
        const float inv = 1.0f / sum;
        *(uint32_t*)(out + (size_t)b * width + h * 64 + dp * 2) = pack_bf16x2(a0 * inv, a1 * inv);
    }
}

int launch_attention_pooled(const bf16_t* q, const bf16_t* qkv, bf16_t* out, const int* pool_idx, const int* row_start, int items,
                            int tokens, int width, int causal, hipStream_t stream, int force_long) {
    if (items <= 0) return KEMR_OK;
    if (width % 64 != 0 || tokens <= 0 || tokens > KEMR_MAX_VISION_TOKENS)
        KEMR_FAIL(KEMR_ERR_INVALID, "attention (pooled row): bad shape t=%d width=%d", tokens, width);
    if (causal && !pool_idx) KEMR_FAIL(KEMR_ERR_INVALID, "attention (pooled row): the causal form needs the pooled positions");
    ProfScope prof(PROF_ATTENTION, stream);
    const long waves = (long)items * (width / 64);
    constexpr int MAXK_LONG = (KEMR_MAX_VISION_TOKENS + 63) / 64 * 64;
    void (*kern)(const bf16_t*, const bf16_t*, bf16_t*, const int*, const int*, int, int, int, int) =
        tokens <= 320 && !force_long ? attention_pooled_kernel<320> : attention_pooled_kernel<MAXK_LONG>;
    hipLaunchKernelGGL(kern, dim3((unsigned)((waves + 3) / 4)), dim3(256), 0, stream, q, qkv, out, pool_idx, row_start, items, tokens,
                       width, causal);
    KEMR_CHECK_LAUNCH("attention_pooled_kernel");
    return KEMR_OK;
}

int launch_attention_packed(const bf16_t* qkv, bf16_t* out, const int* row_start, int batch, int max_t, int width, hipStream_t stream) {
    if (batch <= 0) return KEMR_OK;
    if (!row_start) KEMR_FAIL(KEMR_ERR_INVALID, "attention: packed rows need row_start");
    if (width % 64 != 0 || max_t <= 0) KEMR_FAIL(KEMR_ERR_INVALID, "attention: bad shape t=%d width=%d", max_t, width);
    if (batch > 65528) KEMR_FAIL(KEMR_ERR_INVALID, "attention: batch %d > 65528 (grid.y, rounded up to a multiple of 8)", batch);
    switch ((max_t + 31) / 32) {
        case 1: return launch_nt<1>(qkv, out, batch, max_t, width, 1, stream, row_start);
        case 2: return launch_nt<2>(qkv, out, batch, max_t, width, 1, stream, row_start);
        case 3: return launch_nt<3>(qkv, out, batch, max_t, width, 1, stream, row_start);
        case 4: return launch_nt<4>(qkv, out, batch, max_t, width, 1, stream, row_start);
    }
    KEMR_FAIL(KEMR_ERR_INVALID, "attention: packed rows support lengths up to 128, got %d", max_t);
}

}
```

knowledge_enhanced_multimodal_retrieval_amd/csrc/common.h:

```cpp
#pragma once
#include <hip/hip_runtime.h>
#include <stdint.h>
#include <stddef.h>
#include "../../include/kemr.h"

namespace kemr {

typedef uint16_t bf16_t;
typedef __attribute__((ext_vector_type(8))) short bf16x8;
typedef __attribute__((ext_vector_type(4))) short bf16x4;
typedef __attribute__((ext_vector_type(4))) float f32x4;

void set_error(const char* fmt, ...);
#define KEMR_FAIL(code, ...) do { ::kemr::set_error(__VA_ARGS__); return (code); } while (0)
#define KEMR_CHECK_HIP(expr) do { hipError_t e_ = (expr); if (e_ != hipSuccess) { \
    ::kemr::set_error("%s failed: %s (%s:%d)", #expr, hipGetErrorString(e_), __FILE__, __LINE__); \
    return KEMR_ERR_HIP; } } while (0)
#define KEMR_CHECK_LAUNCH(what) do { hipError_t e_ = hipGetLastError(); if (e_ != hipSuccess) { \
    ::kemr::set_error("launch of %s failed: %s (%s:%d)", what, hipGetErrorString(e_), __FILE__, __LINE__); \
    return KEMR_ERR_HIP; } } while (0)
#define KEMR_TRY(expr) do { int r_ = (expr); if (r_ != KEMR_OK) return r_; } while (0)

static inline uint16_t f32_to_bf16_host(float f) {
    uint32_t u; __builtin_memcpy(&u, &f, 4);
    if ((u & 0x7fffffffu) > 0x7f800000u) return (uint16_t)((u >> 16) | 0x40);
    return (uint16_t)((u + 0x7fffu + ((u >> 16) & 1u)) >> 16);
}
static inline int64_t round_up(int64_t x, int64_t m) { return (x + m - 1) / m * m; }
static inline uint8_t f32_to_e4m3_host(float f) {
    if (f != f) return 0x7f;
    const uint8_t sign = f < 0 ? 0x80 : 0;
    float a = f < 0 ? -f : f;
    if (a >= 448.f) return sign | 0x7e;
    if (a < 0.0009765625f) return sign;
    int e;
    (void)__builtin_frexpf(a, &e);
    e -= 1;
    if (e < -6) {
        const float q = a * 512.f;
        int m = (int)__builtin_nearbyintf(q);
        return sign | (uint8_t)m;
    }
    int m = (int)__builtin_nearbyintf(__builtin_ldexpf(a, 3 - e));
    if (m == 16) { m = 8; e += 1; }
    if (e > 8 || (e == 8 && m > 14)) return sign | 0x7e;
    return sign | (uint8_t)(((e + 7) << 3) | (m - 8));
}

__device__ __forceinline__ float bf16_to_f32(bf16_t b) { return __uint_as_float(((uint32_t)b) << 16); }

constexpr int KEMR_F24 = 24;
struct __attribute__((packed)) f24_t { uint8_t b[3]; };
__device__ __forceinline__ float f24_to_f32(bf16_t hi, uint8_t lo) { return __uint_as_float(((uint32_t)hi << 16) | ((uint32_t)lo << 8)); }
__device__ __forceinline__ uint32_t f32_to_f24_bits(float f) { return __float_as_uint(f) + 0x80u; }
__device__ __forceinline__ bf16_t f32_to_bf16(float f) {
    uint32_t u = __float_as_uint(f);
    return (bf16_t)((u + 0x7fffu + ((u >> 16) & 1u)) >> 16);
}
typedef __bf16 kemr_bf16x2_t __attribute__((ext_vector_type(2)));
typedef float kemr_f32x2_t __attribute__((ext_vector_type(2)));
__device__ __forceinline__ uint32_t pack_bf16x2(float lo, float hi) {
    const kemr_f32x2_t v = {lo, hi};
    return __builtin_bit_cast(uint32_t, __builtin_convertvector(v, kemr_bf16x2_t));
}
__device__ __forceinline__ float quick_gelu(float v) {
    return v * __builtin_amdgcn_rcpf(1.0f + __builtin_amdgcn_exp2f(-1.702f * 1.4426950408889634f * v));
}
typedef float __attribute__((ext_vector_type(2))) f32x2_t;
__device__ __forceinline__ f32x2_t quick_gelu2(f32x2_t v) {
    const f32x2_t t = v * (-1.702f * 1.4426950408889634f);
    f32x2_t e;
    e.x = __builtin_amdgcn_exp2f(t.x);
    e.y = __builtin_amdgcn_exp2f(t.y);
    const f32x2_t d = e + 1.0f;
    f32x2_t r;
    r.x = __builtin_amdgcn_rcpf(d.x);
    r.y = __builtin_amdgcn_rcpf(d.y);
    return v * r;
}
__device__ __forceinline__ float wave_sum(float v) {
#pragma unroll
    for (int o = 32; o > 0; o >>= 1) v += __shfl_xor(v, o);
    return v;
}
__device__ __forceinline__ float wave_max(float v) {
#pragma unroll
    for (int o = 32; o > 0; o >>= 1) v = fmaxf(v, __shfl_xor(v, o));
    return v;
}

enum ProfClass : int { PROF_GEMM = 0, PROF_LAYERNORM = 1, PROF_ATTENTION = 2, PROF_OTHER = 3, PROF_SIM = 4, PROF_NCLASS = 5 };
struct ProfScope {
    ProfScope(int cls, hipStream_t s);
    ~ProfScope();
    int slot; hipStream_t stream;
};

enum GemmEpi : int {
    EPI_BIAS_BF16 = KEMR_EPI_BIAS_BF16,
    EPI_BIAS_QGELU_BF16 = KEMR_EPI_BIAS_QGELU_BF16,
    EPI_BIAS_RESID_F32 = KEMR_EPI_BIAS_RESID_F32,
    EPI_PATCH_F32 = 3,
    EPI_BIAS_RESADD_BF16 = KEMR_EPI_BIAS_RESADD_BF16,
};
struct GemmParams {
    const bf16_t* A;
    const bf16_t* W;
    const float* bias;
    const float* wscale;
    void* C;
    const float* pos;
    int M, N, K;
    int lda, ldw, ldc;
    int patches;
    int dbg;
    int c_rows_padded;
    int order;
    unsigned* stamps;
    const int32_t* sim_gt;
    const float* sim_sgt;
    int32_t* sim_ahead;
    int sim_ng, sim_gbase;
    int sim_nchunks, sim_tpc;
    int sim_xcd;
    const float* simk_taud;
    float* simk_scores;
    int32_t* simk_base;
    int32_t* simk_count;
    int32_t* simk_flag;
    int simk_cap;
};
extern int g_gemm_dbg;
extern int g_gemm_order;
extern int g_sim_lists;
extern int g_attn_xcd;
extern int g_attn_waves;
extern int g_attn_v;
extern int g_gemm_kl;
extern int g_ln_nt;
extern int g_gemm_grid;
extern int g_gemm_conc;
int gemm_read_stamps(unsigned* host_out, int n_words);
int launch_gemm256u_simgmax(const bf16_t* q_panel, int nq, const bf16_t* g_panel, int ng, int kdim, int stride, float* out,
                            hipStream_t stream, bool* used);
struct SimkPlan { int nchunks, tpc, cap; size_t scores_bytes, base_bytes, count_bytes; };
int gemm256u_simk_plan(int nq, int ng, int kdim, double hits_per_query, double spread, SimkPlan* plan, bool* ok);
int launch_gemm256u_simk(const bf16_t* q_panel, int nq, const bf16_t* g_panel, int ng, int kdim, long long gallery_offset,
                         const int32_t* gt_idx, const float* gt_score, int32_t* ahead, const float* taud, const SimkPlan& plan,
                         float* rec_scores, int32_t* rec_base, int32_t* rec_count, int32_t* flag, hipStream_t stream);
int launch_gemm(const GemmParams& p, int epi, hipStream_t stream);
int launch_gemm256(const GemmParams& p, int epi, hipStream_t stream);
int launch_gemm256p(const GemmParams& p, int epi, hipStream_t stream);
int launch_gemm256q(const GemmParams& p, int epi, hipStream_t stream);
int launch_gemm256u(const GemmParams& p, int epi, hipStream_t stream);
bool gemm256u_fits(const GemmParams& p, int elem_size, int c_elem_size = 2);
int launch_gemm256u_simrank(const bf16_t* q_panel, int nq, const bf16_t* g_panel, int ng, int kdim, long long gallery_offset,
                            const int32_t* gt_idx, const float* gt_score, int32_t* ahead, hipStream_t stream, bool* used);
int launch_gemm256u_fp8(const GemmParams& p, int epi, hipStream_t stream);
int launch_gemm256r(const GemmParams& p, int epi, hipStream_t stream);
int launch_gemm_skinny(const GemmParams& p, int epi, hipStream_t stream);
int launch_gemm256w(const GemmParams& p, int epi, hipStream_t stream);
extern int g_gemm_variant;

int launch_select_topk(const float* scores, const int32_t* idx, int nq, int n, long long ld, long long id_offset, int k,
                       float* top_scores, int32_t* top_idx, hipStream_t stream, const int32_t* gt_idx = nullptr,
                       const float* gt_score = nullptr, int32_t* ahead = nullptr);
int launch_layernorm(void* x, int x_dtype, const bf16_t* delta, const bf16_t* delta2, int writeback, const float* gamma,
                     const float* beta, void* y, int rows, int width, int out_dtype, hipStream_t stream);
int launch_attention(const bf16_t* qkv, bf16_t* out, int batch, int t, int width, int causal, hipStream_t stream);
int launch_attention_long(const bf16_t* qkv, bf16_t* out, int batch, int t, int width, hipStream_t stream);
int launch_attention_packed(const bf16_t* qkv, bf16_t* out, const int* row_start, int batch, int max_t, int width, hipStream_t stream);
int launch_im2col(const float* pixels, bf16_t* patches, int batch, int image_size, int patch, int kpad, hipStream_t stream);
int launch_cls_rows(float* x, const float* class_emb, const float* pos, int batch, int tokens, int width, hipStream_t stream);
int launch_pool_index(const int32_t* ids, const int* row_start, int batch, int tokens, int* pool_idx, hipStream_t stream);
int launch_gather_pooled(const void* x, int x_dtype, const void* h, int h_dtype , const int* pool_idx, int batch,
                         int width, void* xc, void* hc, hipStream_t stream);
int launch_attention_pooled(const bf16_t* q, const bf16_t* qkv, bf16_t* out, const int* pool_idx, const int* row_start, int items,
                            int tokens, int width, int causal, hipStream_t stream, int force_long = 0);
int launch_row_starts(const int32_t* lens, int batch, int max_len, int rows, int* row_start, hipStream_t stream);
int launch_text_embed(const int32_t* ids, const float* tok_emb, const float* pos, void* x, int x_dtype, int batch, int ctx,
                      int width, int vocab, hipStream_t stream, const int* row_start = nullptr, int rows = 0);
int launch_tail(const void* x, int x_dtype, const bf16_t* delta, const bf16_t* delta2, const int32_t* ids, int batch, int tokens, int width, const float* gamma,
                const float* beta, const float* proj, int d, int normalize, float* out, hipStream_t stream, const int* row_start = nullptr);

}
```

knowledge_enhanced_multimodal_retrieval_amd/csrc/embed.hip:

```cpp
#include "common.h"

namespace kemr {

__global__ __launch_bounds__(256) void im2col_kernel(const float* __restrict__ px, bf16_t* __restrict__ out,
                                                     int image_size, int patch, int grid, int kpad, int kvalid,
                                                     long long total_pairs) {
    const long long gid = (long long)blockIdx.x * 256 + threadIdx.x;
    if (gid >= total_pairs) return;
    const int kp2 = kpad >> 1;
    const long long row = gid / kp2;
    const int k = (int)(gid - row * kp2) * 2;
    const int P = grid * grid;
    const int b = (int)(row / P), pi = (int)(row - (long long)b * P);
    const int py = pi / grid, pxi = pi - py * grid;
    float v[2];
#pragma unroll
    for (int e = 0; e < 2; ++e) {
        const int kk = k + e;
        if (kk < kvalid) {
            const int c = kk / (patch * patch), rem = kk - c * patch * patch;
            const int dy = rem / patch, dx = rem - dy * patch;
            v[e] = px[(((size_t)b * 3 + c) * image_size + (py * patch + dy)) * image_size + pxi * patch + dx];
        } else {
            v[e] = 0.f;
        }
    }
    *(uint32_t*)(out + (size_t)row * kpad + k) = pack_bf16x2(v[0], v[1]);
}

int launch_im2col(const float* pixels, bf16_t* patches, int batch, int image_size, int patch, int kpad, hipStream_t stream) {
    const int grid = image_size / patch;
    const long long pairs = (long long)batch * grid * grid * (kpad / 2);
    if (pairs <= 0) return KEMR_OK;
    const long long blocks = (pairs + 255) / 256;
    if (blocks > 0x7fffffffLL) KEMR_FAIL(KEMR_ERR_INVALID, "im2col: batch too large");
    ProfScope prof(PROF_OTHER, stream);
    hipLaunchKernelGGL(im2col_kernel, dim3((unsigned)blocks), dim3(256), 0, stream, pixels, patches, image_size, patch,
                       grid, kpad, 3 * patch * patch, pairs);
    KEMR_CHECK_LAUNCH("im2col_kernel");
    return KEMR_OK;
}

__global__ __launch_bounds__(256) void cls_rows_kernel(float* __restrict__ x, const float* __restrict__ cls,
                                                       const float* __restrict__ pos, int tokens, int width) {
    const int b = blockIdx.x;
    float* dst = x + (size_t)b * tokens * width;
    for (int i = threadIdx.x; i < width; i += 256) dst[i] = cls[i] + pos[i];
}

int launch_cls_rows(float* x, const float* class_emb, const float* pos, int batch, int tokens, int width, hipStream_t stream) {
    if (batch <= 0) return KEMR_OK;
    ProfScope prof(PROF_OTHER, stream);
    hipLaunchKernelGGL(cls_rows_kernel, dim3(batch), dim3(256), 0, stream, x, class_emb, pos, tokens, width);
    KEMR_CHECK_LAUNCH("cls_rows_kernel");
    return KEMR_OK;
}

__global__ __launch_bounds__(1024) void row_starts_kernel(const int32_t* __restrict__ lens, int batch, int max_len, int rows,
                                                          int* __restrict__ row_start) {
    __shared__ int part[1024];
    const int tid = threadIdx.x, per = (batch + 1023) / 1024;
    const int i0 = tid * per, i1 = i0 + per < batch ? i0 + per : batch;
    int sum = 0;
    for (int i = i0; i < i1; ++i) { const int l = lens[i]; sum += l < 1 ? 1 : (l > max_len ? max_len : l); }
    part[tid] = sum;
    __syncthreads();
    for (int o = 1; o < 1024; o <<= 1) {
        const int v = tid >= o ? part[tid - o] : 0;
        __syncthreads();
        part[tid] += v;
        __syncthreads();
    }
    int run = part[tid] - sum;
    if (tid == 0) row_start[0] = 0;
    for (int i = i0; i < i1; ++i) {
        const int l = lens[i];
        run += l < 1 ? 1 : (l > max_len ? max_len : l);
        const int cap = rows - (batch - (i + 1));
        row_start[i + 1] = run < cap ? run : cap;
    }
}

int launch_row_starts(const int32_t* lens, int batch, int max_len, int rows, int* row_start, hipStream_t stream) {
    if (batch <= 0) return KEMR_OK;
    if (batch > 65535) KEMR_FAIL(KEMR_ERR_INVALID, "row_starts: batch %d > 65535", batch);
    if (rows < batch || (int64_t)rows > (int64_t)batch * max_len) KEMR_FAIL(KEMR_ERR_INVALID, "row_starts: %d rows for %d texts of 1 .. %d positions", rows, batch, max_len);
    ProfScope prof(PROF_OTHER, stream);
    hipLaunchKernelGGL(row_starts_kernel, dim3(1), dim3(1024), 0, stream, lens, batch, max_len, rows, row_start);
    KEMR_CHECK_LAUNCH("row_starts_kernel");
    return KEMR_OK;
}

template <typename XT>
__global__ __launch_bounds__(256) void text_embed_kernel(const int32_t* __restrict__ ids, const float* __restrict__ tok,
                                                         const float* __restrict__ pos, XT* __restrict__ x,
                                                         int ctx, int width, int vocab, long long total4,
                                                         const int* __restrict__ row_start, int batch) {
    const long long gid = (long long)blockIdx.x * 256 + threadIdx.x;
    if (gid >= total4) return;
    const int w4 = width >> 2;
    const long long row = gid / w4;
    const int c4 = (int)(gid - row * w4);
    int t = (int)(row % ctx);
    long long src = row;
    if (row_start) {
        int lo = 0, hi = batch - 1;
        while (lo < hi) {
            const int mid = (lo + hi + 1) >> 1;
            if (row_start[mid] <= row) lo = mid; else hi = mid - 1;
        }
        t = (int)(row - row_start[lo]);
        t = t < ctx ? t : ctx - 1;
        src = (long long)lo * ctx + t;
    }
    int id = ids[src];
    id = id < 0 ? 0 : (id >= vocab ? vocab - 1 : id);
    const float4 a = ((const float4*)(tok + (size_t)id * width))[c4];
    const float4 p = ((const float4*)(pos + (size_t)t * width))[c4];
    if constexpr (sizeof(XT) == 4) {
        ((float4*)(x + (size_t)row * width))[c4] = make_float4(a.x + p.x, a.y + p.y, a.z + p.z, a.w + p.w);
    } else if constexpr (sizeof(XT) == 3) {
        const uint32_t e0 = f32_to_f24_bits(a.x + p.x), e1 = f32_to_f24_bits(a.y + p.y), e2 = f32_to_f24_bits(a.z + p.z), e3 = f32_to_f24_bits(a.w + p.w);
        uint8_t* r = (uint8_t*)(x + (size_t)row * width);
        uint2 h;
        h.x = (e0 >> 16) | (e1 & 0xffff0000u);
        h.y = (e2 >> 16) | (e3 & 0xffff0000u);
        ((uint2*)r)[c4] = h;
        ((uint32_t*)(r + 2 * (size_t)width))[c4] = ((e0 >> 8) & 0xff) | (e1 & 0xff00) | ((e2 << 8) & 0xff0000) | ((e3 << 16) & 0xff000000u);
    } else {
        uint2 pk;
        pk.x = pack_bf16x2(a.x + p.x, a.y + p.y);
        pk.y = pack_bf16x2(a.z + p.z, a.w + p.w);
        ((uint2*)(x + (size_t)row * width))[c4] = pk;
    }
}

int launch_text_embed(const int32_t* ids, const float* tok_emb, const float* pos, void* x, int x_dtype, int batch, int ctx,
                      int width, int vocab, hipStream_t stream, const int* row_start, int rows) {
    const long long total4 = (row_start ? (long long)rows : (long long)batch * ctx) * (width / 4);
    if (total4 <= 0) return KEMR_OK;
    ProfScope prof(PROF_OTHER, stream);
    const dim3 grid((unsigned)((total4 + 255) / 256));
    if (x_dtype == KEMR_BF16)
        hipLaunchKernelGGL(text_embed_kernel<bf16_t>, grid, dim3(256), 0, stream, ids, tok_emb, pos, (bf16_t*)x, ctx, width, vocab, total4, row_start, batch);
    else if (x_dtype == KEMR_F24)
        hipLaunchKernelGGL(text_embed_kernel<f24_t>, grid, dim3(256), 0, stream, ids, tok_emb, pos, (f24_t*)x, ctx, width, vocab, total4, row_start, batch);
    else
        hipLaunchKernelGGL(text_embed_kernel<float>, grid, dim3(256), 0, stream, ids, tok_emb, pos, (float*)x, ctx, width, vocab, total4, row_start, batch);
    KEMR_CHECK_LAUNCH("text_embed_kernel");
    return KEMR_OK;
}

__global__ __launch_bounds__(256) void pool_index_kernel(const int32_t* __restrict__ ids, const int* __restrict__ row_start, int batch,
                                                         int tokens, int* __restrict__ pool_idx) {
    const int b = blockIdx.x * 4 + (threadIdx.x >> 6), lane = threadIdx.x & 63;
    if (b >= batch) return;
    int best_t = 0;
    if (ids) {
        int best_v = INT_MIN;
        best_t = INT_MAX;
        for (int t = lane; t < tokens; t += 64) {
            const int v = ids[(size_t)b * tokens + t];
            if (v > best_v) { best_v = v; best_t = t; }
        }
#pragma unroll
        for (int o = 32; o > 0; o >>= 1) {
            const int ov = __shfl_xor(best_v, o), ot = __shfl_xor(best_t, o);
            if (ov > best_v || (ov == best_v && ot < best_t)) { best_v = ov; best_t = ot; }
        }
    }
    if (lane == 0) {
        int row = b * tokens + best_t;
        if (row_start) {
            const int r0 = row_start[b], len = row_start[b + 1] - r0;
            row = r0 + (best_t < len ? best_t : len - 1);
        }
        pool_idx[b] = row;
    }
}

int launch_pool_index(const int32_t* ids, const int* row_start, int batch, int tokens, int* pool_idx, hipStream_t stream) {
    if (batch <= 0) return KEMR_OK;
    ProfScope prof(PROF_OTHER, stream);
    hipLaunchKernelGGL(pool_index_kernel, dim3((batch + 3) / 4), dim3(256), 0, stream, ids, row_start, batch, tokens, pool_idx);
    KEMR_CHECK_LAUNCH("pool_index_kernel");
    return KEMR_OK;
}

__global__ __launch_bounds__(256) void gather_pooled_kernel(const uint8_t* __restrict__ x, int x_bytes, const uint8_t* __restrict__ h, int h_bytes,
                                                            const int* __restrict__ pool_idx, int width, uint8_t* __restrict__ xc,
                                                            uint8_t* __restrict__ hc) {
    const int b = blockIdx.x;
    const size_t row = (size_t)pool_idx[b];
    const int xb = width * x_bytes, hb = width * h_bytes;
    for (int i = threadIdx.x * 4; i < xb; i += 1024) *(uint32_t*)(xc + (size_t)b * xb + i) = *(const uint32_t*)(x + row * xb + i);
    for (int i = threadIdx.x * 4; i < hb; i += 1024) *(uint32_t*)(hc + (size_t)b * hb + i) = *(const uint32_t*)(h + row * hb + i);
}

int launch_gather_pooled(const void* x, int x_dtype, const void* h, int h_dtype, const int* pool_idx, int batch, int width, void* xc, void* hc,
                         hipStream_t stream) {
    if (batch <= 0) return KEMR_OK;
    if (width % 4) KEMR_FAIL(KEMR_ERR_INVALID, "gather: width %d must be a multiple of 4", width);
    ProfScope prof(PROF_OTHER, stream);
    const int xb = x_dtype == KEMR_BF16 ? 2 : (x_dtype == KEMR_F24 ? 3 : 4), hb = h_dtype == KEMR_FP8 ? 1 : 2;
    hipLaunchKernelGGL(gather_pooled_kernel, dim3(batch), dim3(256), 0, stream, (const uint8_t*)x, xb, (const uint8_t*)h, hb, pool_idx, width,
                       (uint8_t*)xc, (uint8_t*)hc);
    KEMR_CHECK_LAUNCH("gather_pooled_kernel");
    return KEMR_OK;
}

__device__ __forceinline__ float block_sum(float v, float* red) {
    v = wave_sum(v);
    __syncthreads();
    if ((threadIdx.x & 63) == 0) red[threadIdx.x >> 6] = v;
    __syncthreads();
    return (red[0] + red[1]) + (red[2] + red[3]);
}

template <typename XT>
__global__ __launch_bounds__(256) void tail_proj_kernel(const XT* __restrict__ x, const bf16_t* __restrict__ delta,
                                                        const bf16_t* __restrict__ delta2, const int32_t* __restrict__ ids,
                                                        int tokens, int width, const float* __restrict__ gamma,
                                                        const float* __restrict__ beta, const float* __restrict__ proj,
                                                        int d, float* __restrict__ out, const int* __restrict__ row_start) {
    extern __shared__ __attribute__((aligned(16))) char smem[];
    float* y = (float*)smem;
    float* red = y + width;
    int* pool = (int*)(red + 4);
    const int b = blockIdx.y, tid = threadIdx.x, lane = tid & 63, wid = tid >> 6;

    if (tid < 64) {
        int best_t = 0;
        if (ids) {
            int best_v = INT_MIN;
            best_t = INT_MAX;
            for (int t = tid; t < tokens; t += 64) {
                const int v = ids[(size_t)b * tokens + t];
                if (v > best_v) { best_v = v; best_t = t; }
            }
#pragma unroll
            for (int o = 32; o > 0; o >>= 1) {
                const int ov = __shfl_xor(best_v, o), ot = __shfl_xor(best_t, o);
                if (ov > best_v || (ov == best_v && ot < best_t)) { best_v = ov; best_t = ot; }
            }
        }
        if (tid == 0) *pool = best_t;
    }
    __syncthreads();
    size_t prow = (size_t)b * tokens + *pool;
    if (row_start) {
        const int r0 = row_start[b], len = row_start[b + 1] - r0;
        prow = (size_t)r0 + (*pool < len ? *pool : len - 1);
    }
    const XT* xr = x + prow * width;
    const bf16_t* dr = delta ? delta + prow * width : nullptr;
    const bf16_t* dr2 = delta2 ? delta2 + prow * width : nullptr;

    float s = 0.f;
    for (int i = tid; i < width; i += 256) {
        float v;
        if constexpr (sizeof(XT) == 4) v = xr[i];
        else if constexpr (sizeof(XT) == 3) v = f24_to_f32(((const bf16_t*)xr)[i], ((const uint8_t*)xr)[2 * (size_t)width + i]);
        else v = bf16_to_f32(xr[i]);
        if (dr) v += bf16_to_f32(dr[i]);
        if (dr2) v += bf16_to_f32(dr2[i]);
        y[i] = v;
        s += v;
    }
    const float mean = block_sum(s, red) / width;
    float q = 0.f;
    for (int i = tid; i < width; i += 256) { const float c = y[i] - mean; q += c * c; }
    const float rstd = 1.0f / sqrtf(block_sum(q, red) / width + 1e-5f);
    for (int i = tid; i < width; i += 256) y[i] = (y[i] - mean) * rstd * gamma[i] + beta[i];
    __syncthreads();

    const int j = blockIdx.x * 64 + wid * 16 + (lane & 3) * 4;
    const int g = lane >> 2;
    float4 acc = make_float4(0.f, 0.f, 0.f, 0.f);
    if (j < d) {
#pragma unroll 8
        for (int i = g; i < width; i += 16) {
            const float yi = y[i];
            const float4 p = *(const float4*)(proj + (size_t)i * d + j);
            acc.x = fmaf(yi, p.x, acc.x); acc.y = fmaf(yi, p.y, acc.y);
            acc.z = fmaf(yi, p.z, acc.z); acc.w = fmaf(yi, p.w, acc.w);
        }
    }
#pragma unroll
    for (int o = 4; o < 64; o <<= 1) {
        acc.x += __shfl_xor(acc.x, o); acc.y += __shfl_xor(acc.y, o);
        acc.z += __shfl_xor(acc.z, o); acc.w += __shfl_xor(acc.w, o);
    }
    if (g == 0 && j < d) *(float4*)(out + (size_t)b * d + j) = acc;
}

__global__ __launch_bounds__(256) void l2norm_rows_kernel(float* __restrict__ x, int rows, int d) {
    const int row = blockIdx.x * 4 + (threadIdx.x >> 6), lane = threadIdx.x & 63;
    if (row >= rows) return;
    float* r = x + (size_t)row * d;
    float s = 0.f;
    for (int i = lane; i < d; i += 64) s += r[i] * r[i];
    const float inv = 1.0f / sqrtf(wave_sum(s));
    for (int i = lane; i < d; i += 64) r[i] *= inv;
}

int launch_tail(const void* x, int x_dtype, const bf16_t* delta, const bf16_t* delta2, const int32_t* ids, int batch, int tokens, int width, const float* gamma,
                const float* beta, const float* proj, int d, int normalize, float* out, hipStream_t stream, const int* row_start) {
    if (batch <= 0) return KEMR_OK;
    if (d % 4 != 0 || d <= 0) KEMR_FAIL(KEMR_ERR_INVALID, "tail: embed_dim %d must be a positive multiple of 4", d);
    if (batch > 65535) KEMR_FAIL(KEMR_ERR_INVALID, "tail: batch %d > 65535", batch);
    const size_t smem = (size_t)width * 4 + 32;
    ProfScope prof(PROF_OTHER, stream);
    const dim3 grid((d + 63) / 64, batch);
    if (x_dtype == KEMR_BF16)
        hipLaunchKernelGGL(tail_proj_kernel<bf16_t>, grid, dim3(256), smem, stream, (const bf16_t*)x, delta, delta2, ids, tokens, width, gamma, beta, proj, d, out, row_start);
    else if (x_dtype == KEMR_F24)
        hipLaunchKernelGGL(tail_proj_kernel<f24_t>, grid, dim3(256), smem, stream, (const f24_t*)x, delta, delta2, ids, tokens, width, gamma, beta, proj, d, out, row_start);
    else
        hipLaunchKernelGGL(tail_proj_kernel<float>, grid, dim3(256), smem, stream, (const float*)x, delta, delta2, ids, tokens, width, gamma, beta, proj, d, out, row_start);
    KEMR_CHECK_LAUNCH("tail_proj_kernel");
    if (normalize) {
        hipLaunchKernelGGL(l2norm_rows_kernel, dim3((batch + 3) / 4), dim3(256), 0, stream, out, batch, d);
        KEMR_CHECK_LAUNCH("l2norm_rows_kernel");
    }
    return KEMR_OK;
}

}
```

knowledge_enhanced_multimodal_retrieval_amd/csrc/layernorm.hip:

```cpp
#include "common.h"

namespace kemr {

__device__ __forceinline__ float4 load_row4(const float* r, int i, int) { return ((const float4*)r)[i]; }
__device__ __forceinline__ float4 load_row4(const f24_t* r, int i, int W) {
    const uint2 h = ((const uint2*)r)[i];
    const uint32_t l = ((const uint32_t*)((const uint8_t*)r + 2 * (size_t)W))[i];
    return make_float4(f24_to_f32((bf16_t)(h.x & 0xffff), (uint8_t)l), f24_to_f32((bf16_t)(h.x >> 16), (uint8_t)(l >> 8)),
                       f24_to_f32((bf16_t)(h.y & 0xffff), (uint8_t)(l >> 16)), f24_to_f32((bf16_t)(h.y >> 16), (uint8_t)(l >> 24)));
}
typedef unsigned u32x2_nt __attribute__((ext_vector_type(2)));
typedef float f32x4_nt __attribute__((ext_vector_type(4)));
__device__ __forceinline__ float4 load_row4_nt(const float* r, int i, int) {
    const f32x4_nt v = __builtin_nontemporal_load((const f32x4_nt*)r + i);
    return make_float4(v.x, v.y, v.z, v.w);
}
__device__ __forceinline__ float4 load_row4_nt(const f24_t* r, int i, int W) {
    const u32x2_nt h = __builtin_nontemporal_load((const u32x2_nt*)r + i);
    const uint32_t l = __builtin_nontemporal_load((const uint32_t*)((const uint8_t*)r + 2 * (size_t)W) + i);
    return make_float4(f24_to_f32((bf16_t)(h.x & 0xffff), (uint8_t)l), f24_to_f32((bf16_t)(h.x >> 16), (uint8_t)(l >> 8)),
                       f24_to_f32((bf16_t)(h.y & 0xffff), (uint8_t)(l >> 16)), f24_to_f32((bf16_t)(h.y >> 16), (uint8_t)(l >> 24)));
}
__device__ __forceinline__ float4 load_row4_nt(const bf16_t* r, int i, int) {
    const u32x2_nt d = __builtin_nontemporal_load((const u32x2_nt*)r + i);
    return make_float4(bf16_to_f32((bf16_t)(d.x & 0xffff)), bf16_to_f32((bf16_t)(d.x >> 16)),
                       bf16_to_f32((bf16_t)(d.y & 0xffff)), bf16_to_f32((bf16_t)(d.y >> 16)));
}
__device__ __forceinline__ void store_row4_nt(float* r, int i, float4 v, int) {
    f32x4_nt t = {v.x, v.y, v.z, v.w};
    __builtin_nontemporal_store(t, (f32x4_nt*)r + i);
}
__device__ __forceinline__ void store_row4_nt(f24_t* r, int i, float4 v, int W) {
    const uint32_t a = f32_to_f24_bits(v.x), b = f32_to_f24_bits(v.y), c = f32_to_f24_bits(v.z), d = f32_to_f24_bits(v.w);
    u32x2_nt h = {(a >> 16) | (b & 0xffff0000u), (c >> 16) | (d & 0xffff0000u)};
    __builtin_nontemporal_store(h, (u32x2_nt*)r + i);
    __builtin_nontemporal_store(((a >> 8) & 0xff) | (b & 0xff00) | ((c << 8) & 0xff0000) | ((d << 16) & 0xff000000u), (uint32_t*)((uint8_t*)r + 2 * (size_t)W) + i);
}
__device__ __forceinline__ void store_row4_nt(bf16_t* r, int i, float4 v, int) {
    u32x2_nt pk = {pack_bf16x2(v.x, v.y), pack_bf16x2(v.z, v.w)};
    __builtin_nontemporal_store(pk, (u32x2_nt*)r + i);
}
__device__ __forceinline__ float4 load_delta4(const bf16_t* r, int i) {
    typedef unsigned u32x2_ __attribute__((ext_vector_type(2)));
    const u32x2_ d = __builtin_nontemporal_load((const u32x2_*)r + i);
    return make_float4(bf16_to_f32((bf16_t)(d.x & 0xffff)), bf16_to_f32((bf16_t)(d.x >> 16)),
                       bf16_to_f32((bf16_t)(d.y & 0xffff)), bf16_to_f32((bf16_t)(d.y >> 16)));
}
__device__ __forceinline__ float4 load_row4(const bf16_t* r, int i, int) {
    const uint2 d = ((const uint2*)r)[i];
    return make_float4(bf16_to_f32((bf16_t)(d.x & 0xffff)), bf16_to_f32((bf16_t)(d.x >> 16)),
                       bf16_to_f32((bf16_t)(d.y & 0xffff)), bf16_to_f32((bf16_t)(d.y >> 16)));
}
__device__ __forceinline__ void store_row4(float* r, int i, float4 v, int) { ((float4*)r)[i] = v; }
__device__ __forceinline__ void store_row4(f24_t* r, int i, float4 v, int W) {
    const uint32_t a = f32_to_f24_bits(v.x), b = f32_to_f24_bits(v.y), c = f32_to_f24_bits(v.z), d = f32_to_f24_bits(v.w);
    uint2 h;
    h.x = (a >> 16) | (b & 0xffff0000u);
    h.y = (c >> 16) | (d & 0xffff0000u);
    ((uint2*)r)[i] = h;
    ((uint32_t*)((uint8_t*)r + 2 * (size_t)W))[i] = ((a >> 8) & 0xff) | (b & 0xff00) | ((c << 8) & 0xff0000) | ((d << 16) & 0xff000000u);
}
__device__ __forceinline__ void store_row4(bf16_t* r, int i, float4 v, int) {
    uint2 pk;
    pk.x = pack_bf16x2(v.x, v.y);
    pk.y = pack_bf16x2(v.z, v.w);
    ((uint2*)r)[i] = pk;
}

struct fp8_t { uint8_t v; };
__device__ __forceinline__ void store_row4(fp8_t* r, int i, float4 v, int) {
    const float lim = 448.f;
    int pk = __builtin_amdgcn_cvt_pk_fp8_f32(__builtin_amdgcn_fmed3f(v.x, -lim, lim), __builtin_amdgcn_fmed3f(v.y, -lim, lim), 0, false);
    pk = __builtin_amdgcn_cvt_pk_fp8_f32(__builtin_amdgcn_fmed3f(v.z, -lim, lim), __builtin_amdgcn_fmed3f(v.w, -lim, lim), pk, true);
    ((int*)r)[i] = pk;
}

template <int NV, typename XT, typename OutT, int MODE, int NTD = 3>
__global__ __launch_bounds__(256) void layernorm_kernel(XT* x, const bf16_t* __restrict__ delta, const bf16_t* __restrict__ delta2,
                                                        const float* __restrict__ gamma, const float* __restrict__ beta,
                                                        OutT* y, int rows, float eps) {
    constexpr int W = NV * 256;
    const int lane = threadIdx.x & 63;
    const int row = blockIdx.x * 4 + (threadIdx.x >> 6);
    if (row >= rows) return;
    XT* xr = x + (size_t)row * W;
    float4 v[NV];
    float s = 0.f;
#pragma unroll
    for (int i = 0; i < NV; ++i) {
        v[i] = NTD >= 2 ? load_row4_nt(xr, i * 64 + lane, W) : load_row4(xr, i * 64 + lane, W);
        if constexpr (MODE != 0) {
            const float4 d = NTD >= 1 ? load_delta4(delta + (size_t)row * W, i * 64 + lane) : load_row4(delta + (size_t)row * W, i * 64 + lane, W);
            v[i].x += d.x; v[i].y += d.y; v[i].z += d.z; v[i].w += d.w;
            if (MODE == 1 && delta2) {
                const float4 e = NTD >= 1 ? load_delta4(delta2 + (size_t)row * W, i * 64 + lane) : load_row4(delta2 + (size_t)row * W, i * 64 + lane, W);
                v[i].x += e.x; v[i].y += e.y; v[i].z += e.z; v[i].w += e.w;
            }
            if constexpr (MODE == 1) {
                if constexpr (NTD >= 3) store_row4_nt(xr, i * 64 + lane, v[i], W);
                else store_row4(xr, i * 64 + lane, v[i], W);
            }
        }
        s += (v[i].x + v[i].y) + (v[i].z + v[i].w);
    }
    const float mean = wave_sum(s) * (1.0f / W);
    float q = 0.f;
#pragma unroll
    for (int i = 0; i < NV; ++i) {
        v[i].x -= mean; v[i].y -= mean; v[i].z -= mean; v[i].w -= mean;
        q += (v[i].x * v[i].x + v[i].y * v[i].y) + (v[i].z * v[i].z + v[i].w * v[i].w);
    }
    const float rstd = 1.0f / sqrtf(wave_sum(q) * (1.0f / W) + eps);
#pragma unroll
    for (int i = 0; i < NV; ++i) {
        const float4 g = ((const float4*)gamma)[i * 64 + lane];
        const float4 b = ((const float4*)beta)[i * 64 + lane];
        float4 o;
        o.x = v[i].x * rstd * g.x + b.x;
        o.y = v[i].y * rstd * g.y + b.y;
        o.z = v[i].z * rstd * g.z + b.z;
        o.w = v[i].w * rstd * g.w + b.w;
        store_row4(y + (size_t)row * W, i * 64 + lane, o, W);
    }
}

int g_ln_nt = 3;

template <int NV, typename XT>
static int launch_nv(XT* x, const bf16_t* d1, const bf16_t* d2, int writeback, const float* g, const float* b, void* y, int rows,
                     int out_dtype, hipStream_t s) {
    const int blocks = (rows + 3) / 4;
    ProfScope prof(PROF_LAYERNORM, s);
    if (d1 && writeback && out_dtype == KEMR_FP8)
        hipLaunchKernelGGL((layernorm_kernel<NV, XT, fp8_t, 1>), dim3(blocks), dim3(256), 0, s, x, d1, d2, g, b, (fp8_t*)y, rows, 1e-5f);
    else if (d1 && out_dtype == KEMR_FP8)
        hipLaunchKernelGGL((layernorm_kernel<NV, XT, fp8_t, 2>), dim3(blocks), dim3(256), 0, s, x, d1, d2, g, b, (fp8_t*)y, rows, 1e-5f);
    else if (out_dtype == KEMR_FP8)
        hipLaunchKernelGGL((layernorm_kernel<NV, XT, fp8_t, 0>), dim3(blocks), dim3(256), 0, s, x, d1, d2, g, b, (fp8_t*)y, rows, 1e-5f);
#ifdef KEMR_AB_VARIANTS
    else if (d1 && writeback && g_ln_nt == 0)
        hipLaunchKernelGGL((layernorm_kernel<NV, XT, bf16_t, 1, 0>), dim3(blocks), dim3(256), 0, s, x, d1, d2, g, b, (bf16_t*)y, rows, 1e-5f);
    else if (d1 && g_ln_nt == 0)
        hipLaunchKernelGGL((layernorm_kernel<NV, XT, bf16_t, 2, 0>), dim3(blocks), dim3(256), 0, s, x, d1, d2, g, b, (bf16_t*)y, rows, 1e-5f);
    else if (d1 && writeback && g_ln_nt == 1)
        hipLaunchKernelGGL((layernorm_kernel<NV, XT, bf16_t, 1, 1>), dim3(blocks), dim3(256), 0, s, x, d1, d2, g, b, (bf16_t*)y, rows, 1e-5f);
    else if (d1 && g_ln_nt == 1)
        hipLaunchKernelGGL((layernorm_kernel<NV, XT, bf16_t, 2, 1>), dim3(blocks), dim3(256), 0, s, x, d1, d2, g, b, (bf16_t*)y, rows, 1e-5f);
    else if (d1 && writeback && g_ln_nt == 2)
        hipLaunchKernelGGL((layernorm_kernel<NV, XT, bf16_t, 1, 2>), dim3(blocks), dim3(256), 0, s, x, d1, d2, g, b, (bf16_t*)y, rows, 1e-5f);
#endif
    else if (d1 && writeback)
        hipLaunchKernelGGL((layernorm_kernel<NV, XT, bf16_t, 1>), dim3(blocks), dim3(256), 0, s, x, d1, d2, g, b, (bf16_t*)y, rows, 1e-5f);
    else if (d1)
        hipLaunchKernelGGL((layernorm_kernel<NV, XT, bf16_t, 2>), dim3(blocks), dim3(256), 0, s, x, d1, d2, g, b, (bf16_t*)y, rows, 1e-5f);
    else if (out_dtype == KEMR_BF16)
        hipLaunchKernelGGL((layernorm_kernel<NV, XT, bf16_t, 0>), dim3(blocks), dim3(256), 0, s, x, d1, d2, g, b, (bf16_t*)y, rows, 1e-5f);
    else if (out_dtype == KEMR_F24) {
        if constexpr (sizeof(XT) == 4)
            hipLaunchKernelGGL((layernorm_kernel<NV, XT, f24_t, 0>), dim3(blocks), dim3(256), 0, s, x, d1, d2, g, b, (f24_t*)y, rows, 1e-5f);
        else
            KEMR_FAIL(KEMR_ERR_INVALID, "layernorm: 24-bit output rows need fp32 input rows");
    } else
        hipLaunchKernelGGL((layernorm_kernel<NV, XT, float, 0>), dim3(blocks), dim3(256), 0, s, x, d1, d2, g, b, (float*)y, rows, 1e-5f);
    KEMR_CHECK_LAUNCH("layernorm_kernel");
    return KEMR_OK;
}

template <typename XT>
static int launch_xt(XT* x, const bf16_t* d1, const bf16_t* d2, int writeback, const float* gamma, const float* beta, void* y,
                     int rows, int width, int out_dtype, hipStream_t stream) {
    switch (width) {
        case 256:  return launch_nv<1>(x, d1, d2, writeback, gamma, beta, y, rows, out_dtype, stream);
        case 512:  return launch_nv<2>(x, d1, d2, writeback, gamma, beta, y, rows, out_dtype, stream);
        case 768:  return launch_nv<3>(x, d1, d2, writeback, gamma, beta, y, rows, out_dtype, stream);
        case 1024: return launch_nv<4>(x, d1, d2, writeback, gamma, beta, y, rows, out_dtype, stream);
        case 1280: return launch_nv<5>(x, d1, d2, writeback, gamma, beta, y, rows, out_dtype, stream);
    }
    KEMR_FAIL(KEMR_ERR_INVALID, "layernorm: width %d not in {256,512,768,1024,1280}", width);
}

int launch_layernorm(void* x, int x_dtype, const bf16_t* delta, const bf16_t* delta2, int writeback, const float* gamma,
                     const float* beta, void* y, int rows, int width, int out_dtype, hipStream_t stream) {
    if (rows <= 0) return KEMR_OK;
    if (out_dtype != KEMR_BF16 && out_dtype != KEMR_F32 && out_dtype != KEMR_FP8 && out_dtype != KEMR_F24) KEMR_FAIL(KEMR_ERR_INVALID, "layernorm: bad out dtype %d", out_dtype);
    if (x_dtype != KEMR_BF16 && x_dtype != KEMR_F32 && x_dtype != KEMR_F24) KEMR_FAIL(KEMR_ERR_INVALID, "layernorm: bad row dtype %d", x_dtype);
    if (delta && (out_dtype == KEMR_F32 || out_dtype == KEMR_F24)) KEMR_FAIL(KEMR_ERR_INVALID, "layernorm: the residual forms write bf16 or fp8");
    if (delta2 && !(delta && writeback)) KEMR_FAIL(KEMR_ERR_INVALID, "layernorm: a second delta needs the first one and writeback");
    if (x_dtype == KEMR_BF16) return launch_xt((bf16_t*)x, delta, delta2, writeback, gamma, beta, y, rows, width, out_dtype, stream);
    if (x_dtype == KEMR_F24) return launch_xt((f24_t*)x, delta, delta2, writeback, gamma, beta, y, rows, width, out_dtype, stream);
    return launch_xt((float*)x, delta, delta2, writeback, gamma, beta, y, rows, width, out_dtype, stream);
}

}
```

knowledge_enhanced_multimodal_retrieval_amd/debug.py:

```python
from __future__ import annotations

import contextlib
import ctypes as C

from . import _lib

KEYS = ("gemm_variant", "gemm_flags", "gemm_order", "gemm_grid", "gemm_conc", "gemm_kl", "attn_v", "attn_xcd", "attn_waves", "sim_lists", "ln_nt")


def ab_variants() -> bool:
    return get("ab_variants") == 1


def set(key: str, value: int) -> None:
    _lib.check(_lib.lib().kemr_debug_set(key.encode(), int(value)), f"debug_set({key})")


def get(key: str) -> int:
    v = C.c_int(0)
    _lib.check(_lib.lib().kemr_debug_get(key.encode(), C.byref(v)), f"debug_get({key})")
    return v.value


@contextlib.contextmanager
def override(**kv):
    old = {k: get(k) for k in kv}
    try:
        for k, v in kv.items():
            set(k, v)
        yield
    finally:
        for k, v in old.items():
            set(k, v)


def set_gemm_variant(packed: int) -> None:
    set("gemm_variant", packed & 0xff)
    set("gemm_flags", (packed >> 8) & 0xff)
    if (packed >> 16) & 0xf:
        set("gemm_order", ((packed >> 16) & 0xf) - 1)
    if (packed >> 20) & 0x3:
        set("gemm_conc", ((packed >> 20) & 0x3) - 1)
    if (packed >> 24) & 0xf:
        set("attn_waves", ((packed >> 24) & 0xf) - 1)


def sim_lists(workspace, nq: int, ng: int, kdim: int, k: int):
    out = (C.c_int32 * 6)()
    _lib.check(_lib.lib().kemr_debug_sim_lists(C.c_void_p(workspace.data_ptr()), nq, ng, kdim, k, C.cast(out, C.c_void_p)),
               "debug_sim_lists")
    return list(out)


def gemm_stamps(n_words: int):
    buf = (C.c_uint * n_words)()
    _lib.check(_lib.lib().kemr_debug_gemm_stamps(buf, n_words), "debug_gemm_stamps")
    return buf


def _ptr(t):
    return C.c_void_p(t.data_ptr()) if t is not None else None


def _stream(device):
    import torch
    return C.c_void_p(torch.cuda.current_stream(device).cuda_stream)


def op_attention_packed(qkv, row_start, max_t: int, width: int):
    import torch
    out = torch.zeros((qkv.shape[0], width), dtype=torch.bfloat16, device=qkv.device)
    with torch.cuda.device(qkv.device):
        _lib.check(_lib.lib().kemr_debug_op_attention_packed(_ptr(qkv), _ptr(out), _ptr(row_start), row_start.numel() - 1, max_t,
                                                             width, _stream(qkv.device)), "debug_op_attention_packed")
    return out


def op_attention_pooled(q, qkv, pool_idx, row_start, tokens: int, causal: bool, force_long: bool = False):
    import torch
    items, width = q.shape
    out = torch.zeros((items, width), dtype=torch.bfloat16, device=q.device)
    with torch.cuda.device(q.device):
        _lib.check(_lib.lib().kemr_debug_op_attention_pooled(_ptr(q), _ptr(qkv), _ptr(out), _ptr(pool_idx), _ptr(row_start), items,
                                                             tokens, width, 1 if causal else 0, 1 if force_long else 0,
                                                             _stream(q.device)), "debug_op_attention_pooled")
    return out


def op_tail(x, x_dtype: int, delta, delta2, ids, row_start, batch: int, tokens: int, width: int, gamma, beta, proj,
            normalize: bool):
    import torch
    d = proj.shape[1]
    out = torch.zeros((batch, d), dtype=torch.float32, device=x.device)
    with torch.cuda.device(x.device):
        _lib.check(_lib.lib().kemr_debug_op_tail(_ptr(x), x_dtype, _ptr(delta), _ptr(delta2), _ptr(ids), _ptr(row_start), batch,
                                                 tokens, width, _ptr(gamma), _ptr(beta), _ptr(proj), d, 1 if normalize else 0,
                                                 _ptr(out), _stream(x.device)), "debug_op_tail")
    return out


def _front_workspace(eng, need: int, fill: int):
    import torch
    return torch.full((max(need, 256),), fill, dtype=torch.uint8, device=eng.device)


def image_tokens(eng, pixels, fill: int = 0xff):
    import torch
    a = eng.arch
    batch = pixels.shape[0]
    pixels = pixels.to(device=eng.device, dtype=torch.float32).contiguous()
    out = torch.empty((batch * a.v_tokens, a.v_width), dtype=torch.float32, device=eng.device)
    ws = _front_workspace(eng, int(_lib.lib().kemr_workspace_bytes(eng._h, _lib.TOWER_VISION, batch)), fill)
    with torch.cuda.device(eng.device):
        _lib.check(_lib.lib().kemr_debug_image_tokens(eng._h, _ptr(pixels), batch, _ptr(out), _ptr(ws), ws.numel(),
                                                      _stream(eng.device)), "debug_image_tokens")
    return out


def residual_dtype(eng) -> int:
    v = C.c_int(0)
    _lib.check(_lib.lib().kemr_model_get_option(eng._h, b"precision_residual_bf16", C.byref(v)), "model_get_option")
    if v.value:
        return _lib.KEMR_BF16
    _lib.check(_lib.lib().kemr_model_get_option(eng._h, b"residual_stream_24bit", C.byref(v)), "model_get_option")
    return _lib.KEMR_F24 if v.value else _lib.KEMR_F32


def text_tokens(eng, ids, lens=None, rows: int = 0, fill: int = 0xff):
    import torch
    a = eng.arch
    batch = ids.shape[0]
    ids = ids.to(device=eng.device, dtype=torch.int32).contiguous()
    L = _lib.lib()
    if lens is None:
        n, need, lens_d, rs = batch * a.ctx, int(L.kemr_workspace_bytes(eng._h, _lib.TOWER_TEXT, batch)), None, None
    else:
        lens_d = torch.as_tensor(lens).to(device=eng.device, dtype=torch.int32).contiguous()
        n, need = rows, int(L.kemr_text_packed_workspace_bytes(eng._h, rows, batch))
        rs = torch.full((batch + 1,), -1, dtype=torch.int32, device=eng.device)
    dt = residual_dtype(eng)
    if dt == _lib.KEMR_F24:
        out = torch.empty((n, 3 * a.t_width), dtype=torch.uint8, device=eng.device)
    else:
        out = torch.empty((n, a.t_width), dtype=torch.bfloat16 if dt == _lib.KEMR_BF16 else torch.float32, device=eng.device)
    ws = _front_workspace(eng, need, fill)
    with torch.cuda.device(eng.device):
        _lib.check(L.kemr_debug_text_tokens(eng._h, _ptr(ids), _ptr(lens_d), rows, batch, _ptr(out), _ptr(rs), _ptr(ws), ws.numel(),
                                            _stream(eng.device)), "debug_text_tokens")
    return out, rs
```

Before: 18750 items/s.

## Fuse ln_pre with first ln1 and skip residual writeback in pooled last layer

Adds a layernorm_pair kernel that applies ln_pre and layer 0's ln1 in one pass for the vision tower, so one full read of the residual stream is dropped. In the pooled last layer, ln1 no longer writes the residual back; the deltas are folded in later when gather_pooled picks out the pooled rows, which avoids a full-width write. It also caches hipFuncSetAttribute per kernel and device in the attention launcher, and rewrites im2col and the row load/store helpers. A new ln_fuse knob, on by default, gates the fusion.

```diff
diff --git a/include/kemr_debug.h b/include/kemr_debug.h
--- a/include/kemr_debug.h
+++ b/include/kemr_debug.h
@@ -23,6 +23,14 @@
                        const int* row_start_dev, int batch, int tokens, int width, const float* gamma_dev, const float* beta_dev,
                        const float* proj_dev, int d, int normalize, float* out_dev, void* stream);
 
+int kemr_debug_op_im2col(const float* pixels_dev, void* patches_dev, int batch, int image_size, int patch, int kpad, void* stream);
+int kemr_debug_op_layernorm_pair(const float* x32_dev, const float* gamma0_dev, const float* beta0_dev, void* x_dev, int x_dtype,
+                                 const float* gamma1_dev, const float* beta1_dev, void* h_dev, int rows, int width, void* stream);
+int kemr_debug_op_layernorm_nowb(const void* x_dev, int x_dtype, const void* delta_dev, const void* delta2_dev, const float* gamma_dev,
+                                 const float* beta_dev, void* y_dev, int rows, int width, void* stream);
+int kemr_debug_op_gather_pooled(const void* x_dev, int x_dtype, const void* delta_dev, const void* delta2_dev, const void* h_dev,
+                                const int* pool_idx_dev, int items, int width, void* xc_dev, void* hc_dev, void* stream);
+
 int kemr_debug_image_tokens(struct kemr_model* m, const float* pixels_dev, int batch, float* out_dev, void* workspace_dev,
                             size_t workspace_bytes, void* stream);
 int kemr_debug_text_tokens(struct kemr_model* m, const int32_t* ids_dev, const int32_t* lens_dev, int rows, int batch, void* out_dev,
diff --git a/knowledge_enhanced_multimodal_retrieval_amd/_lib.py b/knowledge_enhanced_multimodal_retrieval_amd/_lib.py
--- a/knowledge_enhanced_multimodal_retrieval_amd/_lib.py
+++ b/knowledge_enhanced_multimodal_retrieval_amd/_lib.py
@@ -86,6 +86,10 @@
     "kemr_debug_op_attention_packed": (_i, [_vp, _vp, _vp, _i, _i, _i, _vp]),
     "kemr_debug_op_attention_pooled": (_i, [_vp, _vp, _vp, _vp, _vp, _i, _i, _i, _i, _i, _vp]),
     "kemr_debug_op_tail": (_i, [_vp, _i, _vp, _vp, _vp, _vp, _i, _i, _i, _vp, _vp, _vp, _i, _i, _vp, _vp]),
+    "kemr_debug_op_im2col": (_i, [_vp, _vp, _i, _i, _i, _i, _vp]),
+    "kemr_debug_op_layernorm_pair": (_i, [_vp, _vp, _vp, _vp, _i, _vp, _vp, _vp, _i, _i, _vp]),
+    "kemr_debug_op_layernorm_nowb": (_i, [_vp, _i, _vp, _vp, _vp, _vp, _vp, _i, _i, _vp]),
+    "kemr_debug_op_gather_pooled": (_i, [_vp, _i, _vp, _vp, _vp, _vp, _i, _i, _vp, _vp, _vp]),
     "kemr_debug_image_tokens": (_i, [_vp, _vp, _i, _vp, _vp, _sz, _vp]),
     "kemr_debug_text_tokens": (_i, [_vp, _vp, _vp, _i, _i, _vp, _vp, _vp, _sz, _vp]),
 }
diff --git a/knowledge_enhanced_multimodal_retrieval_amd/csrc/api.hip b/knowledge_enhanced_multimodal_retrieval_amd/csrc/api.hip
--- a/knowledge_enhanced_multimodal_retrieval_amd/csrc/api.hip
+++ b/knowledge_enhanced_multimodal_retrieval_amd/csrc/api.hip
@@ -338,6 +338,8 @@
 
 namespace {
 
+int g_ln_fuse = 1;
+
 struct Workspace {
     void* x;
     int x_dtype;
@@ -394,7 +396,8 @@
 }
 
 int run_blocks(const TowerW& t, const Workspace& w, int batch, int causal, int fp8, int want_resadd, hipStream_t s, bool* pending,
-               const int* row_start = nullptr, int rows = 0, int last_pooled = 0, const int32_t* ids = nullptr, bool* compact = nullptr) {
+               const int* row_start = nullptr, int rows = 0, int last_pooled = 0, const int32_t* ids = nullptr, bool* compact = nullptr,
+               bool ln1_done = false) {
     const int W = t.width, M = row_start ? rows : batch * t.tokens;
     const bool fq = fp8 & 1, f1 = fp8 & 2;
     bool resadd = want_resadd >= (w.x_dtype == KEMR_BF16 ? 1 : 2) && M > 512 && W % 256 == 0 && w.x_dtype != KEMR_F24;
@@ -413,13 +416,14 @@
     for (int l = 0; l < t.layers; ++l) {
         const LayerW& L = t.layer[l];
         if (pooled && l == t.layers - 1) {
-            KEMR_TRY(launch_layernorm(w.x, w.x_dtype, l ? w.delta : nullptr, l ? w.delta2 : nullptr, 1, L.ln1_g, L.ln1_b, w.h, M, W, fq ? KEMR_FP8 : KEMR_BF16, s));
+            if (l && g_ln_fuse) KEMR_TRY(launch_layernorm_nowb(w.x, w.x_dtype, w.delta, w.delta2, L.ln1_g, L.ln1_b, w.h, M, W, fq ? KEMR_FP8 : KEMR_BF16, s));
+            else if (l || !ln1_done) KEMR_TRY(launch_layernorm(w.x, w.x_dtype, l ? w.delta : nullptr, l ? w.delta2 : nullptr, 1, L.ln1_g, L.ln1_b, w.h, M, W, fq ? KEMR_FP8 : KEMR_BF16, s));
             GemmParams g{};
             g.c_rows_padded = 1;
             g.M = M; g.A = w.h; g.lda = W; g.ldw = W; g.bias = L.bqkv + W; g.C = w.big + W; g.ldc = 3 * W; g.N = 2 * W; g.K = W;
             if (fq) { g.W = (const bf16_t*)(L.wqkv8 + (size_t)W * W); g.wscale = L.sqkv + W; KEMR_TRY(launch_gemm256u_fp8(g, EPI_BIAS_BF16, s)); }
             else { g.W = L.wqkv + (size_t)W * W; KEMR_TRY(launch_gemm(g, EPI_BIAS_BF16, s)); }
-            KEMR_TRY(launch_gather_pooled(w.x, w.x_dtype, w.h, fq ? KEMR_FP8 : KEMR_BF16, w.pool_idx, batch, W, w.xc, w.hc, s));
+            KEMR_TRY(launch_gather_pooled(w.x, w.x_dtype, w.h, fq ? KEMR_FP8 : KEMR_BF16, w.pool_idx, batch, W, w.xc, w.hc, s, l && g_ln_fuse ? w.delta : nullptr, l && g_ln_fuse ? w.delta2 : nullptr));
             g.M = batch; g.A = w.hc; g.bias = L.bqkv; g.C = w.qc; g.ldc = W; g.N = W;
             if (fq) { g.W = (const bf16_t*)L.wqkv8; g.wscale = L.sqkv; KEMR_TRY(launch_gemm256u_fp8(g, EPI_BIAS_BF16, s)); g.wscale = nullptr; }
             else { g.W = L.wqkv; KEMR_TRY(launch_gemm(g, EPI_BIAS_BF16, s)); }
@@ -433,7 +437,8 @@
             KEMR_TRY(launch_gemm(g, EPI_BIAS_BF16, s));
             break;
         }
-        if (resadd) KEMR_TRY(launch_layernorm(w.x, w.x_dtype, nullptr, nullptr, 0, L.ln1_g, L.ln1_b, w.h, M, W, fq ? KEMR_FP8 : KEMR_BF16, s));
+        if (l == 0 && ln1_done) {}
+        else if (resadd) KEMR_TRY(launch_layernorm(w.x, w.x_dtype, nullptr, nullptr, 0, L.ln1_g, L.ln1_b, w.h, M, W, fq ? KEMR_FP8 : KEMR_BF16, s));
         else KEMR_TRY(launch_layernorm(w.x, w.x_dtype, l ? w.delta : nullptr, l ? w.delta2 : nullptr, 1, L.ln1_g, L.ln1_b, w.h, M, W, fq ? KEMR_FP8 : KEMR_BF16, s));
         GemmParams g{};
         g.M = M;
@@ -525,9 +530,11 @@
     KEMR_TRY(image_front(m, pixels_dev, batch, out_dev, workspace_dev, workspace_bytes, s, "encode_image", w));
     if (batch == 0) return KEMR_OK;
     const int W = m->cfg.v_width, T = m->patches + 1;
-    KEMR_TRY(launch_layernorm(w.x32, KEMR_F32, nullptr, nullptr, 0, m->lnpre_g, m->lnpre_b, w.x, batch * T, W, w.x_dtype, s));
+    const bool pair = m->vis.layers > 0 && !(m->fp8 & 1) && g_ln_fuse;
+    if (pair) KEMR_TRY(launch_layernorm_pair(w.x32, m->lnpre_g, m->lnpre_b, w.x, w.x_dtype, m->vis.layer[0].ln1_g, m->vis.layer[0].ln1_b, w.h, batch * T, W, s));
+    else KEMR_TRY(launch_layernorm(w.x32, KEMR_F32, nullptr, nullptr, 0, m->lnpre_g, m->lnpre_b, w.x, batch * T, W, w.x_dtype, s));
     bool vb = false, vc = false;
-    KEMR_TRY(run_blocks(m->vis, w, batch, 0, m->fp8, m->resadd, s, &vb, nullptr, 0, m->last_pooled, nullptr, &vc));
+    KEMR_TRY(run_blocks(m->vis, w, batch, 0, m->fp8, m->resadd, s, &vb, nullptr, 0, m->last_pooled, nullptr, &vc, pair));
     if (vc) KEMR_TRY(launch_tail(w.xc, w.x_dtype, w.d1c, w.d2c, nullptr, batch, 1, W, m->lnpost_g, m->lnpost_b, m->vproj, m->cfg.embed_dim, normalize, out_dev, s));
     else KEMR_TRY(launch_tail(w.x, w.x_dtype, vb ? w.delta : nullptr, vb ? w.delta2 : nullptr, nullptr, batch, T, W, m->lnpost_g, m->lnpost_b, m->vproj, m->cfg.embed_dim, normalize, out_dev, s));
     return KEMR_OK;
@@ -613,6 +620,8 @@
         {"attn_xcd", &g_attn_xcd, 0, 1, ~0u},
         {"attn_waves", &g_attn_waves, 0, 8, 1u << 0},
         {"ln_nt", &g_ln_nt, 0, 3, 1u << 3},
+        {"ln_fuse", &g_ln_fuse, 0, 1, ~0u},
+        {"tail_rows", &g_tail_rows, 0, 16, ~0u},
         {"sim_lists", sim_lists_knob(), 0, 3, ~0u},
         {"ab_variants", &g_ab_variants, -1, -2, 0},
     };
@@ -675,6 +684,32 @@
                        proj_dev, d, normalize, out_dev, (hipStream_t)stream, row_start_dev);
 }
 
+extern "C" int kemr_debug_op_im2col(const float* pixels_dev, void* patches_dev, int batch, int image_size, int patch, int kpad, void* stream) {
+    if (!pixels_dev || !patches_dev) KEMR_FAIL(KEMR_ERR_INVALID, "debug_op_im2col: null argument");
+    return launch_im2col(pixels_dev, (bf16_t*)patches_dev, batch, image_size, patch, kpad, (hipStream_t)stream);
+}
+
+extern "C" int kemr_debug_op_layernorm_pair(const float* x32_dev, const float* gamma0_dev, const float* beta0_dev, void* x_dev, int x_dtype,
+                                            const float* gamma1_dev, const float* beta1_dev, void* h_dev, int rows, int width, void* stream) {
+    if (!x32_dev || !gamma0_dev || !beta0_dev || !x_dev || !gamma1_dev || !beta1_dev || !h_dev) KEMR_FAIL(KEMR_ERR_INVALID, "debug_op_layernorm_pair: null argument");
+    return launch_layernorm_pair(x32_dev, gamma0_dev, beta0_dev, x_dev, x_dtype, gamma1_dev, beta1_dev, (bf16_t*)h_dev, rows, width, (hipStream_t)stream);
+}
+
+extern "C" int kemr_debug_op_layernorm_nowb(const void* x_dev, int x_dtype, const void* delta_dev, const void* delta2_dev, const float* gamma_dev,
+                                            const float* beta_dev, void* y_dev, int rows, int width, void* stream) {
+    if (!x_dev || !delta_dev || !gamma_dev || !beta_dev || !y_dev) KEMR_FAIL(KEMR_ERR_INVALID, "debug_op_layernorm_nowb: null argument");
+    return launch_layernorm_nowb(x_dev, x_dtype, (const bf16_t*)delta_dev, (const bf16_t*)delta2_dev, gamma_dev, beta_dev, y_dev, rows, width, KEMR_BF16,
+                                 (hipStream_t)stream);
+}
+
+extern "C" int kemr_debug_op_gather_pooled(const void* x_dev, int x_dtype, const void* delta_dev, const void* delta2_dev, const void* h_dev,
+                                           const int* pool_idx_dev, int items, int width, void* xc_dev, void* hc_dev, void* stream) {
+    if (!x_dev || !h_dev || !pool_idx_dev || !xc_dev || !hc_dev) KEMR_FAIL(KEMR_ERR_INVALID, "debug_op_gather_pooled: null argument");
+    if (x_dtype != KEMR_F32 && x_dtype != KEMR_BF16 && x_dtype != KEMR_F24) KEMR_FAIL(KEMR_ERR_INVALID, "debug_op_gather_pooled: bad row dtype %d", x_dtype);
+    return launch_gather_pooled(x_dev, x_dtype, h_dev, KEMR_BF16, pool_idx_dev, items, width, xc_dev, hc_dev, (hipStream_t)stream,
+                                (const bf16_t*)delta_dev, (const bf16_t*)delta2_dev);
+}
+
 extern "C" int kemr_debug_image_tokens(kemr_model* m, const float* pixels_dev, int batch, float* out_dev, void* workspace_dev,
                                        size_t workspace_bytes, void* stream) {
     hipStream_t s = (hipStream_t)stream;
diff --git a/knowledge_enhanced_multimodal_retrieval_amd/csrc/attention.hip b/knowledge_enhanced_multimodal_retrieval_amd/csrc/attention.hip
--- a/knowledge_enhanced_multimodal_retrieval_amd/csrc/attention.hip
+++ b/knowledge_enhanced_multimodal_retrieval_amd/csrc/attention.hip
@@ -285,7 +285,15 @@
     } else {
         kern = attention_kernel<NT32, false, 0>;
     }
-    KEMR_CHECK_HIP(hipFuncSetAttribute((const void*)kern, hipFuncAttributeMaxDynamicSharedMemorySize, smem));
+    static struct { const void* kern; unsigned devices; } done[8];
+    int dev = 0;
+    KEMR_CHECK_HIP(hipGetDevice(&dev));
+    int slot = 0;
+    while (slot < 8 && done[slot].kern && done[slot].kern != (const void*)kern) ++slot;
+    if (slot == 8 || dev >= 32 || !((done[slot].devices >> dev) & 1u)) {
+        KEMR_CHECK_HIP(hipFuncSetAttribute((const void*)kern, hipFuncAttributeMaxDynamicSharedMemorySize, smem));
+        if (slot < 8 && dev < 32) { done[slot].kern = (const void*)kern; done[slot].devices |= 1u << dev; }
+    }
     hipLaunchKernelGGL(kern, xgrid, dim3(threads), smem, stream, qkv, out, t, width, xbatch, row_start);
     KEMR_CHECK_LAUNCH("attention_kernel");
     return KEMR_OK;
diff --git a/knowledge_enhanced_multimodal_retrieval_amd/csrc/common.h b/knowledge_enhanced_multimodal_retrieval_amd/csrc/common.h
--- a/knowledge_enhanced_multimodal_retrieval_amd/csrc/common.h
+++ b/knowledge_enhanced_multimodal_retrieval_amd/csrc/common.h
@@ -62,6 +62,33 @@
 __device__ __forceinline__ uint32_t pack_bf16x2(float lo, float hi) {
     const kemr_f32x2_t v = {lo, hi};
     return __builtin_bit_cast(uint32_t, __builtin_convertvector(v, kemr_bf16x2_t));
+}
+__device__ __forceinline__ float4 load_row4(const float* r, int i, int) { return ((const float4*)r)[i]; }
+__device__ __forceinline__ float4 load_row4(const f24_t* r, int i, int W) {
+    const uint2 h = ((const uint2*)r)[i];
+    const uint32_t l = ((const uint32_t*)((const uint8_t*)r + 2 * (size_t)W))[i];
+    return make_float4(f24_to_f32((bf16_t)(h.x & 0xffff), (uint8_t)l), f24_to_f32((bf16_t)(h.x >> 16), (uint8_t)(l >> 8)),
+                       f24_to_f32((bf16_t)(h.y & 0xffff), (uint8_t)(l >> 16)), f24_to_f32((bf16_t)(h.y >> 16), (uint8_t)(l >> 24)));
+}
+__device__ __forceinline__ float4 load_row4(const bf16_t* r, int i, int) {
+    const uint2 d = ((const uint2*)r)[i];
+    return make_float4(bf16_to_f32((bf16_t)(d.x & 0xffff)), bf16_to_f32((bf16_t)(d.x >> 16)),
+                       bf16_to_f32((bf16_t)(d.y & 0xffff)), bf16_to_f32((bf16_t)(d.y >> 16)));
+}
+__device__ __forceinline__ void store_row4(float* r, int i, float4 v, int) { ((float4*)r)[i] = v; }
+__device__ __forceinline__ void store_row4(f24_t* r, int i, float4 v, int W) {
+    const uint32_t a = f32_to_f24_bits(v.x), b = f32_to_f24_bits(v.y), c = f32_to_f24_bits(v.z), d = f32_to_f24_bits(v.w);
+    uint2 h;
+    h.x = (a >> 16) | (b & 0xffff0000u);
+    h.y = (c >> 16) | (d & 0xffff0000u);
+    ((uint2*)r)[i] = h;
+    ((uint32_t*)((uint8_t*)r + 2 * (size_t)W))[i] = ((a >> 8) & 0xff) | (b & 0xff00) | ((c << 8) & 0xff0000) | ((d << 16) & 0xff000000u);
+}
+__device__ __forceinline__ void store_row4(bf16_t* r, int i, float4 v, int) {
+    uint2 pk;
+    pk.x = pack_bf16x2(v.x, v.y);
+    pk.y = pack_bf16x2(v.z, v.w);
+    ((uint2*)r)[i] = pk;
 }
 __device__ __forceinline__ float quick_gelu(float v) {
     return v * __builtin_amdgcn_rcpf(1.0f + __builtin_amdgcn_exp2f(-1.702f * 1.4426950408889634f * v));
@@ -138,6 +165,7 @@
 extern int g_attn_v;
 extern int g_gemm_kl;
 extern int g_ln_nt;
+extern int g_tail_rows;
 extern int g_gemm_grid;
 extern int g_gemm_conc;
 int gemm_read_stamps(unsigned* host_out, int n_words);
@@ -167,6 +195,10 @@
                        const float* gt_score = nullptr, int32_t* ahead = nullptr);
 int launch_layernorm(void* x, int x_dtype, const bf16_t* delta, const bf16_t* delta2, int writeback, const float* gamma,
                      const float* beta, void* y, int rows, int width, int out_dtype, hipStream_t stream);
+int launch_layernorm_nowb(const void* x, int x_dtype, const bf16_t* delta, const bf16_t* delta2, const float* gamma, const float* beta,
+                          void* y, int rows, int width, int out_dtype, hipStream_t stream);
+int launch_layernorm_pair(const float* x32, const float* g0, const float* b0, void* x, int x_dtype, const float* g1, const float* b1,
+                          bf16_t* h, int rows, int width, hipStream_t stream);
 int launch_attention(const bf16_t* qkv, bf16_t* out, int batch, int t, int width, int causal, hipStream_t stream);
 int launch_attention_long(const bf16_t* qkv, bf16_t* out, int batch, int t, int width, hipStream_t stream);
 int launch_attention_packed(const bf16_t* qkv, bf16_t* out, const int* row_start, int batch, int max_t, int width, hipStream_t stream);
@@ -174,7 +206,7 @@
 int launch_cls_rows(float* x, const float* class_emb, const float* pos, int batch, int tokens, int width, hipStream_t stream);
 int launch_pool_index(const int32_t* ids, const int* row_start, int batch, int tokens, int* pool_idx, hipStream_t stream);
 int launch_gather_pooled(const void* x, int x_dtype, const void* h, int h_dtype , const int* pool_idx, int batch,
-                         int width, void* xc, void* hc, hipStream_t stream);
+                         int width, void* xc, void* hc, hipStream_t stream, const bf16_t* delta = nullptr, const bf16_t* delta2 = nullptr);
 int launch_attention_pooled(const bf16_t* q, const bf16_t* qkv, bf16_t* out, const int* pool_idx, const int* row_start, int items,
                             int tokens, int width, int causal, hipStream_t stream, int force_long = 0);
 int launch_row_starts(const int32_t* lens, int batch, int max_len, int rows, int* row_start, hipStream_t stream);
diff --git a/knowledge_enhanced_multimodal_retrieval_amd/csrc/embed.hip b/knowledge_enhanced_multimodal_retrieval_amd/csrc/embed.hip
--- a/knowledge_enhanced_multimodal_retrieval_amd/csrc/embed.hip
+++ b/knowledge_enhanced_multimodal_retrieval_amd/csrc/embed.hip
@@ -2,41 +2,77 @@
 
 namespace kemr {
 
-__global__ __launch_bounds__(256) void im2col_kernel(const float* __restrict__ px, bf16_t* __restrict__ out,
-                                                     int image_size, int patch, int grid, int kpad, int kvalid,
-                                                     long long total_pairs) {
-    const long long gid = (long long)blockIdx.x * 256 + threadIdx.x;
-    if (gid >= total_pairs) return;
-    const int kp2 = kpad >> 1;
-    const long long row = gid / kp2;
-    const int k = (int)(gid - row * kp2) * 2;
-    const int P = grid * grid;
-    const int b = (int)(row / P), pi = (int)(row - (long long)b * P);
-    const int py = pi / grid, pxi = pi - py * grid;
-    float v[2];
-#pragma unroll
-    for (int e = 0; e < 2; ++e) {
-        const int kk = k + e;
-        if (kk < kvalid) {
-            const int c = kk / (patch * patch), rem = kk - c * patch * patch;
-            const int dy = rem / patch, dx = rem - dy * patch;
-            v[e] = px[(((size_t)b * 3 + c) * image_size + (py * patch + dy)) * image_size + pxi * patch + dx];
-        } else {
-            v[e] = 0.f;
-        }
-    }
-    *(uint32_t*)(out + (size_t)row * kpad + k) = pack_bf16x2(v[0], v[1]);
+constexpr int TAIL_BLOCK_ROWS = 8, TAIL_BLOCK_MIN = 64;
+
+template <bool VEC>
+__global__ __launch_bounds__(256) void im2col_kernel(const float* __restrict__ px, bf16_t* __restrict__ out, int image_size, int patch,
+                                                     int grid, int kpad, int kvalid, int gx, int nchunk) {
+    extern __shared__ __attribute__((aligned(16))) char smem[];
+    bf16_t* rows = (bf16_t*)smem;
+    const int tid = threadIdx.x;
+    const int chunk = blockIdx.x % nchunk, bp = blockIdx.x / nchunk;
+    const int py = bp % grid, b = bp / grid;
+    const int px0 = chunk * gx, n = grid - px0 < gx ? grid - px0 : gx;
+    const int seg = n * patch, lines = 3 * patch;
+    const float* src = px + ((size_t)b * 3 * image_size + (size_t)py * patch) * image_size + (size_t)px0 * patch;
+    const int pad = kpad - kvalid;
+    for (int i = tid; i < n * pad; i += 256) rows[(i / pad) * kpad + kvalid + i % pad] = 0;
+    if constexpr (VEC) {
+        typedef float f32x4_ __attribute__((ext_vector_type(4)));
+        const int q4 = seg >> 2;
+        const bool even = !(patch & 1);
+        for (int i = tid; i < lines * q4; i += 256) {
+            const int line = i / q4, x0 = (i - line * q4) * 4;
+            const int c = line / patch, dy = line - c * patch;
+            const f32x4_ v = __builtin_nontemporal_load((const f32x4_*)(src + ((size_t)c * image_size + dy) * image_size + x0));
+            const int kb = line * patch;
+            if (even) {
+#pragma unroll
+                for (int e = 0; e < 4; e += 2) {
+                    const int g = (x0 + e) / patch, dx = x0 + e - g * patch;
+                    *(uint32_t*)(rows + g * kpad + kb + dx) = pack_bf16x2(v[e], v[e + 1]);
+                }
+            } else {
+#pragma unroll
+                for (int e = 0; e < 4; ++e) {
+                    const int g = (x0 + e) / patch, dx = x0 + e - g * patch;
+                    rows[g * kpad + kb + dx] = (bf16_t)pack_bf16x2(v[e], 0.f);
+                }
+            }
+        }
+    } else {
+        for (int i = tid; i < lines * seg; i += 256) {
+            const int line = i / seg, x = i - line * seg;
+            const int c = line / patch, dy = line - c * patch;
+            const int g = x / patch, dx = x - g * patch;
+            rows[g * kpad + line * patch + dx] = (bf16_t)pack_bf16x2(src[((size_t)c * image_size + dy) * image_size + x], 0.f);
+        }
+    }
+    __syncthreads();
+    uint4* dst = (uint4*)(out + ((size_t)bp * grid + px0) * kpad);
+    for (int i = tid; i < n * (kpad >> 3); i += 256) dst[i] = ((const uint4*)rows)[i];
 }
 
 int launch_im2col(const float* pixels, bf16_t* patches, int batch, int image_size, int patch, int kpad, hipStream_t stream) {
-    const int grid = image_size / patch;
-    const long long pairs = (long long)batch * grid * grid * (kpad / 2);
-    if (pairs <= 0) return KEMR_OK;
-    const long long blocks = (pairs + 255) / 256;
+    if (batch <= 0) return KEMR_OK;
+    if (patch <= 0 || image_size < patch) KEMR_FAIL(KEMR_ERR_INVALID, "im2col: bad image size %d / patch %d", image_size, patch);
+    const int grid = image_size / patch, kvalid = 3 * patch * patch;
+    if (kpad % 8 || kpad < kvalid) KEMR_FAIL(KEMR_ERR_INVALID, "im2col: kpad %d must be a multiple of 8 and >= %d", kpad, kvalid);
+    int gx = (48 << 10) / (kpad * 2);
+    if (gx < 1) KEMR_FAIL(KEMR_ERR_INVALID, "im2col: patch %d too large", patch);
+    if (gx > grid) gx = grid;
+    const int nchunk = (grid + gx - 1) / gx;
+    const long long blocks = (long long)batch * grid * nchunk;
     if (blocks > 0x7fffffffLL) KEMR_FAIL(KEMR_ERR_INVALID, "im2col: batch too large");
-    ProfScope prof(PROF_OTHER, stream);
-    hipLaunchKernelGGL(im2col_kernel, dim3((unsigned)blocks), dim3(256), 0, stream, pixels, patches, image_size, patch,
-                       grid, kpad, 3 * patch * patch, pairs);
+    const bool vec = (uintptr_t)pixels % 16 == 0 && image_size % 4 == 0 && (gx * patch) % 4 == 0 && (grid * patch) % 4 == 0;
+    const size_t smem = (size_t)gx * kpad * 2;
+    ProfScope prof(PROF_OTHER, stream);
+    if (vec)
+        hipLaunchKernelGGL(im2col_kernel<true>, dim3((unsigned)blocks), dim3(256), smem, stream, pixels, patches, image_size, patch, grid, kpad,
+                           kvalid, gx, nchunk);
+    else
+        hipLaunchKernelGGL(im2col_kernel<false>, dim3((unsigned)blocks), dim3(256), smem, stream, pixels, patches, image_size, patch, grid, kpad,
+                           kvalid, gx, nchunk);
     KEMR_CHECK_LAUNCH("im2col_kernel");
     return KEMR_OK;
 }
@@ -197,14 +233,45 @@
     for (int i = threadIdx.x * 4; i < hb; i += 1024) *(uint32_t*)(hc + (size_t)b * hb + i) = *(const uint32_t*)(h + row * hb + i);
 }
 
+template <typename XT>
+__global__ __launch_bounds__(256) void gather_pooled_sum_kernel(const XT* __restrict__ x, const bf16_t* __restrict__ d1, const bf16_t* __restrict__ d2,
+                                                                const uint8_t* __restrict__ h, int h_bytes, const int* __restrict__ pool_idx,
+                                                                int width, XT* __restrict__ xc, uint8_t* __restrict__ hc) {
+    const int b = blockIdx.x;
+    const size_t row = (size_t)pool_idx[b];
+    for (int i = threadIdx.x; i < (width >> 2); i += 256) {
+        float4 v = load_row4(x + row * width, i, width);
+        const float4 d = load_row4(d1 + row * width, i, width);
+        v.x += d.x; v.y += d.y; v.z += d.z; v.w += d.w;
+        if (d2) {
+            const float4 e = load_row4(d2 + row * width, i, width);
+            v.x += e.x; v.y += e.y; v.z += e.z; v.w += e.w;
+        }
+        store_row4(xc + (size_t)b * width, i, v, width);
+    }
+    const int hb = width * h_bytes;
+    for (int i = threadIdx.x * 4; i < hb; i += 1024) *(uint32_t*)(hc + (size_t)b * hb + i) = *(const uint32_t*)(h + row * hb + i);
+}
+
 int launch_gather_pooled(const void* x, int x_dtype, const void* h, int h_dtype, const int* pool_idx, int batch, int width, void* xc, void* hc,
-                         hipStream_t stream) {
+                         hipStream_t stream, const bf16_t* delta, const bf16_t* delta2) {
     if (batch <= 0) return KEMR_OK;
     if (width % 4) KEMR_FAIL(KEMR_ERR_INVALID, "gather: width %d must be a multiple of 4", width);
+    if (delta2 && !delta) KEMR_FAIL(KEMR_ERR_INVALID, "gather: a second delta needs the first one");
     ProfScope prof(PROF_OTHER, stream);
     const int xb = x_dtype == KEMR_BF16 ? 2 : (x_dtype == KEMR_F24 ? 3 : 4), hb = h_dtype == KEMR_FP8 ? 1 : 2;
-    hipLaunchKernelGGL(gather_pooled_kernel, dim3(batch), dim3(256), 0, stream, (const uint8_t*)x, xb, (const uint8_t*)h, hb, pool_idx, width,
-                       (uint8_t*)xc, (uint8_t*)hc);
+    if (!delta)
+        hipLaunchKernelGGL(gather_pooled_kernel, dim3(batch), dim3(256), 0, stream, (const uint8_t*)x, xb, (const uint8_t*)h, hb, pool_idx, width,
+                           (uint8_t*)xc, (uint8_t*)hc);
+    else if (x_dtype == KEMR_BF16)
+        hipLaunchKernelGGL(gather_pooled_sum_kernel<bf16_t>, dim3(batch), dim3(256), 0, stream, (const bf16_t*)x, delta, delta2, (const uint8_t*)h, hb,
+                           pool_idx, width, (bf16_t*)xc, (uint8_t*)hc);
+    else if (x_dtype == KEMR_F24)
+        hipLaunchKernelGGL(gather_pooled_sum_kernel<f24_t>, dim3(batch), dim3(256), 0, stream, (const f24_t*)x, delta, delta2, (const uint8_t*)h, hb,
+                           pool_idx, width, (f24_t*)xc, (uint8_t*)hc);
+    else
+        hipLaunchKernelGGL(gather_pooled_sum_kernel<float>, dim3(batch), dim3(256), 0, stream, (const float*)x, delta, delta2, (const uint8_t*)h, hb,
+                           pool_idx, width, (float*)xc, (uint8_t*)hc);
     KEMR_CHECK_LAUNCH("gather_pooled_kernel");
     return KEMR_OK;
 }
@@ -294,6 +361,98 @@
     if (g == 0 && j < d) *(float4*)(out + (size_t)b * d + j) = acc;
 }
 
+template <typename XT, int ROWS>
+__global__ __launch_bounds__(256) void tail_proj_rows_kernel(const XT* __restrict__ x, const bf16_t* __restrict__ delta,
+                                                             const bf16_t* __restrict__ delta2, const int32_t* __restrict__ ids,
+                                                             int batch, int tokens, int width, const float* __restrict__ gamma,
+                                                             const float* __restrict__ beta, const float* __restrict__ proj,
+                                                             int d, float* __restrict__ out, const int* __restrict__ row_start) {
+    extern __shared__ __attribute__((aligned(16))) char smem[];
+    float* ys = (float*)smem;
+    float* red = ys + (size_t)ROWS * width;
+    int* pool = (int*)(red + 4);
+    const int b0 = blockIdx.y * ROWS, tid = threadIdx.x, lane = tid & 63, wid = tid >> 6;
+    const int nr = batch - b0 < ROWS ? batch - b0 : ROWS;
+
+    for (int r = 0; r < nr; ++r) {
+        const int b = b0 + r;
+        float* y = ys + (size_t)r * width;
+        __syncthreads();
+        if (tid < 64) {
+            int best_t = 0;
+            if (ids) {
+                int best_v = INT_MIN;
+                best_t = INT_MAX;
+                for (int t = tid; t < tokens; t += 64) {
+                    const int v = ids[(size_t)b * tokens + t];
+                    if (v > best_v) { best_v = v; best_t = t; }
+                }
+#pragma unroll
+                for (int o = 32; o > 0; o >>= 1) {
+                    const int ov = __shfl_xor(best_v, o), ot = __shfl_xor(best_t, o);
+                    if (ov > best_v || (ov == best_v && ot < best_t)) { best_v = ov; best_t = ot; }
+                }
+            }
+            if (tid == 0) *pool = best_t;
+        }
+        __syncthreads();
+        size_t prow = (size_t)b * tokens + *pool;
+        if (row_start) {
+            const int r0 = row_start[b], len = row_start[b + 1] - r0;
+            prow = (size_t)r0 + (*pool < len ? *pool : len - 1);
+        }
+        const XT* xr = x + prow * width;
+        const bf16_t* dr = delta ? delta + prow * width : nullptr;
+        const bf16_t* dr2 = delta2 ? delta2 + prow * width : nullptr;
+
+        float s = 0.f;
+        for (int i = tid; i < width; i += 256) {
+            float v;
+            if constexpr (sizeof(XT) == 4) v = xr[i];
+            else if constexpr (sizeof(XT) == 3) v = f24_to_f32(((const bf16_t*)xr)[i], ((const uint8_t*)xr)[2 * (size_t)width + i]);
+            else v = bf16_to_f32(xr[i]);
+            if (dr) v += bf16_to_f32(dr[i]);
+            if (dr2) v += bf16_to_f32(dr2[i]);
+            y[i] = v;
+            s += v;
+        }
+        const float mean = block_sum(s, red) / width;
+        float q = 0.f;
+        for (int i = tid; i < width; i += 256) { const float c = y[i] - mean; q += c * c; }
+        const float rstd = 1.0f / sqrtf(block_sum(q, red) / width + 1e-5f);
+        for (int i = tid; i < width; i += 256) y[i] = (y[i] - mean) * rstd * gamma[i] + beta[i];
+    }
+    for (int i = nr * width + tid; i < ROWS * width; i += 256) ys[i] = 0.f;
+    __syncthreads();
+
+    const int j = blockIdx.x * 64 + wid * 16 + (lane & 3) * 4;
+    const int g = lane >> 2;
+    float4 acc[ROWS];
+#pragma unroll
+    for (int r = 0; r < ROWS; ++r) acc[r] = make_float4(0.f, 0.f, 0.f, 0.f);
+    if (j < d) {
+#pragma unroll 4
+        for (int i = g; i < width; i += 16) {
+            const float4 p = *(const float4*)(proj + (size_t)i * d + j);
+#pragma unroll
+            for (int r = 0; r < ROWS; ++r) {
+                const float yi = ys[r * width + i];
+                acc[r].x = fmaf(yi, p.x, acc[r].x); acc[r].y = fmaf(yi, p.y, acc[r].y);
+                acc[r].z = fmaf(yi, p.z, acc[r].z); acc[r].w = fmaf(yi, p.w, acc[r].w);
+            }
+        }
+    }
+#pragma unroll
+    for (int r = 0; r < ROWS; ++r) {
+#pragma unroll
+        for (int o = 4; o < 64; o <<= 1) {
+            acc[r].x += __shfl_xor(acc[r].x, o); acc[r].y += __shfl_xor(acc[r].y, o);
+            acc[r].z += __shfl_xor(acc[r].z, o); acc[r].w += __shfl_xor(acc[r].w, o);
+        }
+        if (g == 0 && j < d && r < nr) *(float4*)(out + (size_t)(b0 + r) * d + j) = acc[r];
+    }
+}
+
 __global__ __launch_bounds__(256) void l2norm_rows_kernel(float* __restrict__ x, int rows, int d) {
     const int row = blockIdx.x * 4 + (threadIdx.x >> 6), lane = threadIdx.x & 63;
     if (row >= rows) return;
@@ -304,20 +463,36 @@
     for (int i = lane; i < d; i += 64) r[i] *= inv;
 }
 
+int g_tail_rows = 0;
+
+template <typename XT>
+static void launch_tail_xt(int rows, dim3 grid, size_t smem, hipStream_t stream, const XT* x, const bf16_t* delta, const bf16_t* delta2,
+                           const int32_t* ids, int batch, int tokens, int width, const float* gamma, const float* beta, const float* proj, int d,
+                           float* out, const int* row_start) {
+    if (rows == 1)
+        hipLaunchKernelGGL(tail_proj_kernel<XT>, grid, dim3(256), smem, stream, x, delta, delta2, ids, tokens, width, gamma, beta, proj, d, out, row_start);
+    else if (rows == 4)
+        hipLaunchKernelGGL((tail_proj_rows_kernel<XT, 4>), grid, dim3(256), smem, stream, x, delta, delta2, ids, batch, tokens, width, gamma, beta, proj, d, out, row_start);
+    else if (rows == 8)
+        hipLaunchKernelGGL((tail_proj_rows_kernel<XT, 8>), grid, dim3(256), smem, stream, x, delta, delta2, ids, batch, tokens, width, gamma, beta, proj, d, out, row_start);
+    else
+        hipLaunchKernelGGL((tail_proj_rows_kernel<XT, 16>), grid, dim3(256), smem, stream, x, delta, delta2, ids, batch, tokens, width, gamma, beta, proj, d, out, row_start);
+}
+
 int launch_tail(const void* x, int x_dtype, const bf16_t* delta, const bf16_t* delta2, const int32_t* ids, int batch, int tokens, int width, const float* gamma,
                 const float* beta, const float* proj, int d, int normalize, float* out, hipStream_t stream, const int* row_start) {
     if (batch <= 0) return KEMR_OK;
     if (d % 4 != 0 || d <= 0) KEMR_FAIL(KEMR_ERR_INVALID, "tail: embed_dim %d must be a positive multiple of 4", d);
     if (batch > 65535) KEMR_FAIL(KEMR_ERR_INVALID, "tail: batch %d > 65535", batch);
-    const size_t smem = (size_t)width * 4 + 32;
-    ProfScope prof(PROF_OTHER, stream);
-    const dim3 grid((d + 63) / 64, batch);
-    if (x_dtype == KEMR_BF16)
-        hipLaunchKernelGGL(tail_proj_kernel<bf16_t>, grid, dim3(256), smem, stream, (const bf16_t*)x, delta, delta2, ids, tokens, width, gamma, beta, proj, d, out, row_start);
-    else if (x_dtype == KEMR_F24)
-        hipLaunchKernelGGL(tail_proj_kernel<f24_t>, grid, dim3(256), smem, stream, (const f24_t*)x, delta, delta2, ids, tokens, width, gamma, beta, proj, d, out, row_start);
-    else
-        hipLaunchKernelGGL(tail_proj_kernel<float>, grid, dim3(256), smem, stream, (const float*)x, delta, delta2, ids, tokens, width, gamma, beta, proj, d, out, row_start);
+    int rows = g_tail_rows == 0 ? (batch >= TAIL_BLOCK_MIN ? TAIL_BLOCK_ROWS : 1) : (g_tail_rows == 1 ? 1 : (g_tail_rows <= 4 ? 4 : (g_tail_rows <= 8 ? 8 : 16)));
+    while (rows > 4 && (size_t)rows * width * 4 + 32 > (64u << 10)) rows >>= 1;
+    if ((size_t)rows * width * 4 + 32 > (64u << 10)) rows = 1;
+    const size_t smem = (size_t)rows * width * 4 + 32;
+    ProfScope prof(PROF_OTHER, stream);
+    const dim3 grid((d + 63) / 64, (batch + rows - 1) / rows);
+    if (x_dtype == KEMR_BF16) launch_tail_xt(rows, grid, smem, stream, (const bf16_t*)x, delta, delta2, ids, batch, tokens, width, gamma, beta, proj, d, out, row_start);
+    else if (x_dtype == KEMR_F24) launch_tail_xt(rows, grid, smem, stream, (const f24_t*)x, delta, delta2, ids, batch, tokens, width, gamma, beta, proj, d, out, row_start);
+    else launch_tail_xt(rows, grid, smem, stream, (const float*)x, delta, delta2, ids, batch, tokens, width, gamma, beta, proj, d, out, row_start);
     KEMR_CHECK_LAUNCH("tail_proj_kernel");
     if (normalize) {
         hipLaunchKernelGGL(l2norm_rows_kernel, dim3((batch + 3) / 4), dim3(256), 0, stream, out, batch, d);
diff --git a/knowledge_enhanced_multimodal_retrieval_amd/csrc/layernorm.hip b/knowledge_enhanced_multimodal_retrieval_amd/csrc/layernorm.hip
--- a/knowledge_enhanced_multimodal_retrieval_amd/csrc/layernorm.hip
+++ b/knowledge_enhanced_multimodal_retrieval_amd/csrc/layernorm.hip
@@ -2,13 +2,6 @@
 
 namespace kemr {
 
-__device__ __forceinline__ float4 load_row4(const float* r, int i, int) { return ((const float4*)r)[i]; }
-__device__ __forceinline__ float4 load_row4(const f24_t* r, int i, int W) {
-    const uint2 h = ((const uint2*)r)[i];
-    const uint32_t l = ((const uint32_t*)((const uint8_t*)r + 2 * (size_t)W))[i];
-    return make_float4(f24_to_f32((bf16_t)(h.x & 0xffff), (uint8_t)l), f24_to_f32((bf16_t)(h.x >> 16), (uint8_t)(l >> 8)),
-                       f24_to_f32((bf16_t)(h.y & 0xffff), (uint8_t)(l >> 16)), f24_to_f32((bf16_t)(h.y >> 16), (uint8_t)(l >> 24)));
-}
 typedef unsigned u32x2_nt __attribute__((ext_vector_type(2)));
 typedef float f32x4_nt __attribute__((ext_vector_type(4)));
 __device__ __forceinline__ float4 load_row4_nt(const float* r, int i, int) {
@@ -45,26 +38,6 @@
     const u32x2_ d = __builtin_nontemporal_load((const u32x2_*)r + i);
     return make_float4(bf16_to_f32((bf16_t)(d.x & 0xffff)), bf16_to_f32((bf16_t)(d.x >> 16)),
                        bf16_to_f32((bf16_t)(d.y & 0xffff)), bf16_to_f32((bf16_t)(d.y >> 16)));
-}
-__device__ __forceinline__ float4 load_row4(const bf16_t* r, int i, int) {
-    const uint2 d = ((const uint2*)r)[i];
-    return make_float4(bf16_to_f32((bf16_t)(d.x & 0xffff)), bf16_to_f32((bf16_t)(d.x >> 16)),
-                       bf16_to_f32((bf16_t)(d.y & 0xffff)), bf16_to_f32((bf16_t)(d.y >> 16)));
-}
-__device__ __forceinline__ void store_row4(float* r, int i, float4 v, int) { ((float4*)r)[i] = v; }
-__device__ __forceinline__ void store_row4(f24_t* r, int i, float4 v, int W) {
-    const uint32_t a = f32_to_f24_bits(v.x), b = f32_to_f24_bits(v.y), c = f32_to_f24_bits(v.z), d = f32_to_f24_bits(v.w);
-    uint2 h;
-    h.x = (a >> 16) | (b & 0xffff0000u);
-    h.y = (c >> 16) | (d & 0xffff0000u);
-    ((uint2*)r)[i] = h;
-    ((uint32_t*)((uint8_t*)r + 2 * (size_t)W))[i] = ((a >> 8) & 0xff) | (b & 0xff00) | ((c << 8) & 0xff0000) | ((d << 16) & 0xff000000u);
-}
-__device__ __forceinline__ void store_row4(bf16_t* r, int i, float4 v, int) {
-    uint2 pk;
-    pk.x = pack_bf16x2(v.x, v.y);
-    pk.y = pack_bf16x2(v.z, v.w);
-    ((uint2*)r)[i] = pk;
 }
 
 struct fp8_t { uint8_t v; };
@@ -92,7 +65,7 @@
         if constexpr (MODE != 0) {
             const float4 d = NTD >= 1 ? load_delta4(delta + (size_t)row * W, i * 64 + lane) : load_row4(delta + (size_t)row * W, i * 64 + lane, W);
             v[i].x += d.x; v[i].y += d.y; v[i].z += d.z; v[i].w += d.w;
-            if (MODE == 1 && delta2) {
+            if ((MODE == 1 || MODE == 3) && delta2) {
                 const float4 e = NTD >= 1 ? load_delta4(delta2 + (size_t)row * W, i * 64 + lane) : load_row4(delta2 + (size_t)row * W, i * 64 + lane, W);
                 v[i].x += e.x; v[i].y += e.y; v[i].z += e.z; v[i].w += e.w;
             }
@@ -124,6 +97,75 @@
     }
 }
 
+__device__ __forceinline__ float4 stored_row4(float4 v, const float*) { return v; }
+__device__ __forceinline__ float4 stored_row4(float4 v, const f24_t*) {
+    return make_float4(__uint_as_float(f32_to_f24_bits(v.x) & 0xffffff00u), __uint_as_float(f32_to_f24_bits(v.y) & 0xffffff00u),
+                       __uint_as_float(f32_to_f24_bits(v.z) & 0xffffff00u), __uint_as_float(f32_to_f24_bits(v.w) & 0xffffff00u));
+}
+__device__ __forceinline__ float4 stored_row4(float4 v, const bf16_t*) {
+    const uint32_t a = pack_bf16x2(v.x, v.y), b = pack_bf16x2(v.z, v.w);
+    return make_float4(__uint_as_float(a << 16), __uint_as_float(a & 0xffff0000u), __uint_as_float(b << 16), __uint_as_float(b & 0xffff0000u));
+}
+
+template <int NV, typename XT>
+__global__ __launch_bounds__(256) void layernorm_pair_kernel(const float* x32, const float* __restrict__ g0, const float* __restrict__ b0,
+                                                             XT* x, const float* __restrict__ g1, const float* __restrict__ b1,
+                                                             bf16_t* __restrict__ h, int rows, float eps) {
+    constexpr int W = NV * 256;
+    const int lane = threadIdx.x & 63;
+    const int row = blockIdx.x * 4 + (threadIdx.x >> 6);
+    if (row >= rows) return;
+    const float* xr = x32 + (size_t)row * W;
+    float4 v[NV];
+    float s = 0.f;
+#pragma unroll
+    for (int i = 0; i < NV; ++i) {
+        v[i] = load_row4_nt(xr, i * 64 + lane, W);
+        s += (v[i].x + v[i].y) + (v[i].z + v[i].w);
+    }
+    float mean = wave_sum(s) * (1.0f / W);
+    float q = 0.f;
+#pragma unroll
+    for (int i = 0; i < NV; ++i) {
+        v[i].x -= mean; v[i].y -= mean; v[i].z -= mean; v[i].w -= mean;
+        q += (v[i].x * v[i].x + v[i].y * v[i].y) + (v[i].z * v[i].z + v[i].w * v[i].w);
+    }
+    float rstd = 1.0f / sqrtf(wave_sum(q) * (1.0f / W) + eps);
+    s = 0.f;
+#pragma unroll
+    for (int i = 0; i < NV; ++i) {
+        const float4 g = ((const float4*)g0)[i * 64 + lane];
+        const float4 b = ((const float4*)b0)[i * 64 + lane];
+        float4 o;
+        o.x = v[i].x * rstd * g.x + b.x;
+        o.y = v[i].y * rstd * g.y + b.y;
+        o.z = v[i].z * rstd * g.z + b.z;
+        o.w = v[i].w * rstd * g.w + b.w;
+        store_row4_nt(x + (size_t)row * W, i * 64 + lane, o, W);
+        v[i] = stored_row4(o, (const XT*)nullptr);
+        s += (v[i].x + v[i].y) + (v[i].z + v[i].w);
+    }
+    mean = wave_sum(s) * (1.0f / W);
+    q = 0.f;
+#pragma unroll
+    for (int i = 0; i < NV; ++i) {
+        v[i].x -= mean; v[i].y -= mean; v[i].z -= mean; v[i].w -= mean;
+        q += (v[i].x * v[i].x + v[i].y * v[i].y) + (v[i].z * v[i].z + v[i].w * v[i].w);
+    }
+    rstd = 1.0f / sqrtf(wave_sum(q) * (1.0f / W) + eps);
+#pragma unroll
+    for (int i = 0; i < NV; ++i) {
+        const float4 g = ((const float4*)g1)[i * 64 + lane];
+        const float4 b = ((const float4*)b1)[i * 64 + lane];
+        float4 o;
+        o.x = v[i].x * rstd * g.x + b.x;
+        o.y = v[i].y * rstd * g.y + b.y;
+        o.z = v[i].z * rstd * g.z + b.z;
+        o.w = v[i].w * rstd * g.w + b.w;
+        store_row4(h + (size_t)row * W, i * 64 + lane, o, W);
+    }
+}
+
 int g_ln_nt = 3;
 
 template <int NV, typename XT>
@@ -131,7 +173,11 @@
                      int out_dtype, hipStream_t s) {
     const int blocks = (rows + 3) / 4;
     ProfScope prof(PROF_LAYERNORM, s);
-    if (d1 && writeback && out_dtype == KEMR_FP8)
+    if (d1 && writeback == 2 && out_dtype == KEMR_FP8)
+        hipLaunchKernelGGL((layernorm_kernel<NV, XT, fp8_t, 3>), dim3(blocks), dim3(256), 0, s, x, d1, d2, g, b, (fp8_t*)y, rows, 1e-5f);
+    else if (d1 && writeback == 2)
+        hipLaunchKernelGGL((layernorm_kernel<NV, XT, bf16_t, 3>), dim3(blocks), dim3(256), 0, s, x, d1, d2, g, b, (bf16_t*)y, rows, 1e-5f);
+    else if (d1 && writeback && out_dtype == KEMR_FP8)
         hipLaunchKernelGGL((layernorm_kernel<NV, XT, fp8_t, 1>), dim3(blocks), dim3(256), 0, s, x, d1, d2, g, b, (fp8_t*)y, rows, 1e-5f);
     else if (d1 && out_dtype == KEMR_FP8)
         hipLaunchKernelGGL((layernorm_kernel<NV, XT, fp8_t, 2>), dim3(blocks), dim3(256), 0, s, x, d1, d2, g, b, (fp8_t*)y, rows, 1e-5f);
@@ -186,9 +232,47 @@
     if (x_dtype != KEMR_BF16 && x_dtype != KEMR_F32 && x_dtype != KEMR_F24) KEMR_FAIL(KEMR_ERR_INVALID, "layernorm: bad row dtype %d", x_dtype);
     if (delta && (out_dtype == KEMR_F32 || out_dtype == KEMR_F24)) KEMR_FAIL(KEMR_ERR_INVALID, "layernorm: the residual forms write bf16 or fp8");
     if (delta2 && !(delta && writeback)) KEMR_FAIL(KEMR_ERR_INVALID, "layernorm: a second delta needs the first one and writeback");
+    writeback = writeback ? 1 : 0;
     if (x_dtype == KEMR_BF16) return launch_xt((bf16_t*)x, delta, delta2, writeback, gamma, beta, y, rows, width, out_dtype, stream);
     if (x_dtype == KEMR_F24) return launch_xt((f24_t*)x, delta, delta2, writeback, gamma, beta, y, rows, width, out_dtype, stream);
     return launch_xt((float*)x, delta, delta2, writeback, gamma, beta, y, rows, width, out_dtype, stream);
 }
 
-}
+int launch_layernorm_nowb(const void* x, int x_dtype, const bf16_t* delta, const bf16_t* delta2, const float* gamma, const float* beta,
+                          void* y, int rows, int width, int out_dtype, hipStream_t stream) {
+    if (rows <= 0) return KEMR_OK;
+    if (!delta) KEMR_FAIL(KEMR_ERR_INVALID, "layernorm: the form without write-back needs a delta");
+    if (out_dtype != KEMR_BF16 && out_dtype != KEMR_FP8) KEMR_FAIL(KEMR_ERR_INVALID, "layernorm: the residual forms write bf16 or fp8");
+    if (x_dtype == KEMR_BF16) return launch_xt((bf16_t*)x, delta, delta2, 2, gamma, beta, y, rows, width, out_dtype, stream);
+    if (x_dtype == KEMR_F24) return launch_xt((f24_t*)x, delta, delta2, 2, gamma, beta, y, rows, width, out_dtype, stream);
+    if (x_dtype == KEMR_F32) return launch_xt((float*)x, delta, delta2, 2, gamma, beta, y, rows, width, out_dtype, stream);
+    KEMR_FAIL(KEMR_ERR_INVALID, "layernorm: bad row dtype %d", x_dtype);
+}
+
+template <typename XT>
+static int launch_pair_xt(const float* x32, const float* g0, const float* b0, XT* x, const float* g1, const float* b1, bf16_t* h, int rows,
+                          int width, hipStream_t s) {
+    const int blocks = (rows + 3) / 4;
+    ProfScope prof(PROF_LAYERNORM, s);
+    switch (width) {
+        case 256:  hipLaunchKernelGGL((layernorm_pair_kernel<1, XT>), dim3(blocks), dim3(256), 0, s, x32, g0, b0, x, g1, b1, h, rows, 1e-5f); break;
+        case 512:  hipLaunchKernelGGL((layernorm_pair_kernel<2, XT>), dim3(blocks), dim3(256), 0, s, x32, g0, b0, x, g1, b1, h, rows, 1e-5f); break;
+        case 768:  hipLaunchKernelGGL((layernorm_pair_kernel<3, XT>), dim3(blocks), dim3(256), 0, s, x32, g0, b0, x, g1, b1, h, rows, 1e-5f); break;
+        case 1024: hipLaunchKernelGGL((layernorm_pair_kernel<4, XT>), dim3(blocks), dim3(256), 0, s, x32, g0, b0, x, g1, b1, h, rows, 1e-5f); break;
+        case 1280: hipLaunchKernelGGL((layernorm_pair_kernel<5, XT>), dim3(blocks), dim3(256), 0, s, x32, g0, b0, x, g1, b1, h, rows, 1e-5f); break;
+        default: KEMR_FAIL(KEMR_ERR_INVALID, "layernorm: width %d not in {256,512,768,1024,1280}", width);
+    }
+    KEMR_CHECK_LAUNCH("layernorm_pair_kernel");
+    return KEMR_OK;
+}
+
+int launch_layernorm_pair(const float* x32, const float* g0, const float* b0, void* x, int x_dtype, const float* g1, const float* b1,
+                          bf16_t* h, int rows, int width, hipStream_t stream) {
+    if (rows <= 0) return KEMR_OK;
+    if (x_dtype == KEMR_BF16) return launch_pair_xt(x32, g0, b0, (bf16_t*)x, g1, b1, h, rows, width, stream);
+    if (x_dtype == KEMR_F24) return launch_pair_xt(x32, g0, b0, (f24_t*)x, g1, b1, h, rows, width, stream);
+    if (x_dtype == KEMR_F32) return launch_pair_xt(x32, g0, b0, (float*)x, g1, b1, h, rows, width, stream);
+    KEMR_FAIL(KEMR_ERR_INVALID, "layernorm: bad row dtype %d", x_dtype);
+}
+
+}
diff --git a/knowledge_enhanced_multimodal_retrieval_amd/debug.py b/knowledge_enhanced_multimodal_retrieval_amd/debug.py
--- a/knowledge_enhanced_multimodal_retrieval_amd/debug.py
+++ b/knowledge_enhanced_multimodal_retrieval_amd/debug.py
@@ -5,7 +5,7 @@
 
 from . import _lib
 
-KEYS = ("gemm_variant", "gemm_flags", "gemm_order", "gemm_grid", "gemm_conc", "gemm_kl", "attn_v", "attn_xcd", "attn_waves", "sim_lists", "ln_nt")
+KEYS = ("gemm_variant", "gemm_flags", "gemm_order", "gemm_grid", "gemm_conc", "gemm_kl", "attn_v", "attn_xcd", "attn_waves", "sim_lists", "ln_nt", "tail_rows", "ln_fuse")
 
 
 def ab_variants() -> bool:
```

After: 18810 items/s, median of 6. No clear change (+0.3%).
